# Weepingchestnut/SAVSR

Measured on NVIDIA B200. Metric: hr_mpix_per_s, higher is better.
Workload: dtype bf16

## Files before the change

savsr_b200/csrc/common.cuh:

```cuda
#pragma once

#include <cuda.h>
#include <cuda_bf16.h>
#include <cuda_fp16.h>
#include <cuda_runtime.h>
#include <stdint.h>
#include <stdio.h>
#include <string.h>

#include "../../include/savsr_b200.h"

namespace savsr {

void set_error(const char* fmt, ...);
int cuda_fail(cudaError_t e, const char* what);

#define SAVSR_CUDA(expr)                                   \
  do {                                                     \
    cudaError_t _e = (expr);                               \
    if (_e != cudaSuccess) return ::savsr::cuda_fail(_e, #expr); \
  } while (0)

#define SAVSR_REQUIRE(cond, ...)          \
  do {                                    \
    if (!(cond)) {                        \
      ::savsr::set_error(__VA_ARGS__);    \
      return 1;                           \
    }                                     \
  } while (0)

constexpr int kTileW = SAVSR_TILE_W;
constexpr int kTileH = SAVSR_TILE_H;
constexpr int kTileM = kTileW * kTileH;
constexpr int kC = 64;

}

struct savsr_ctx {
  int device;
  int sm_count;
  int cc_major, cc_minor;
  void* encode_tiled;
  int fmt;
  int opt[SAVSR_OPT_COUNT];
  uint32_t attr_mask;
  long long* conv_dbg;
};

namespace savsr {
enum AttrBit { kAttrIgemm = 0 , kAttrBigk = 8, kAttrKsta = 9, kAttrSatuHr = 10, kAttrOsaLinear = 11,
               kAttrFused = 12, kAttrBigk128 = 13, kAttrSatuHrBf16 = 14, kAttrWgrad = 15, kAttrWgradBatched = 16,
               kAttrOsaAssembleTrain = 17, kAttrOsaUnfoldBwd = 18, kAttrOsaChain = 19, kAttrOsaMatvec = 20 ,
               kAttrCaBackward = 23 };
template <class F>
inline int ensure_smem_attr(savsr_ctx* ctx, int bit, F func, size_t bytes) {
  if (ctx->attr_mask & (1u << bit)) return 0;
  SAVSR_CUDA(cudaFuncSetAttribute(func, cudaFuncAttributeMaxDynamicSharedMemorySize, static_cast<int>(bytes)));
  ctx->attr_mask |= 1u << bit;
  return 0;
}
template <class... KArgs, class... Args>
inline cudaError_t launch_k(bool pdl, void (*kernel)(KArgs...), dim3 grid, dim3 block, size_t smem, cudaStream_t st, Args&&... args) {
  cudaLaunchConfig_t cfg = {};
  cfg.gridDim = grid; cfg.blockDim = block; cfg.dynamicSmemBytes = smem; cfg.stream = st;
  cudaLaunchAttribute attr[1];
  attr[0].id = cudaLaunchAttributeProgrammaticStreamSerialization;
  attr[0].val.programmaticStreamSerializationAllowed = 1;
  cfg.attrs = attr; cfg.numAttrs = pdl ? 1 : 0;
  return cudaLaunchKernelEx(&cfg, kernel, static_cast<KArgs>(args)...);
}
struct DeviceGuard {
  int prev = -1;
  bool switched = false;
  explicit DeviceGuard(int device) {
    const bool known = cudaGetDevice(&prev) == cudaSuccess;
    const bool ok = cudaSetDevice(device) == cudaSuccess;
    switched = known && ok && prev != device;
  }
  ~DeviceGuard() { if (switched) cudaSetDevice(prev); }
};
}

struct savsr_arena {
  savsr_ctx* ctx;
  __nv_bfloat16* base;
  int nslots, batch, height, width;
  int tiles_x, tiles_y;
  CUtensorMap tm_tile;
  CUtensorMap tm_halo;
};

#ifdef __CUDACC__
namespace savsr {

__device__ __forceinline__ uint32_t smem_u32(const void* p) {
  return static_cast<uint32_t>(__cvta_generic_to_shared(p));
}

__device__ __forceinline__ uint32_t pack_h2(float lo, float hi, int fmt) {
  if (fmt) {
    __half2 v = __floats2half2_rn(lo, hi);
    return *reinterpret_cast<uint32_t*>(&v);
  }
  __nv_bfloat162 v = __floats2bfloat162_rn(lo, hi);
  return *reinterpret_cast<uint32_t*>(&v);
}
__device__ __forceinline__ float h_lo(uint32_t v, int fmt) {
  return fmt ? __half2float(__ushort_as_half(static_cast<unsigned short>(v & 0xffffu))) : __uint_as_float(v << 16);
}
__device__ __forceinline__ float h_hi(uint32_t v, int fmt) {
  return fmt ? __half2float(__ushort_as_half(static_cast<unsigned short>(v >> 16))) : __uint_as_float(v & 0xffff0000u);
}
__device__ __forceinline__ float h_to_float(uint16_t raw, int fmt) { return h_lo(raw, fmt); }
__device__ __forceinline__ uint16_t float_to_h(float x, int fmt) { return static_cast<uint16_t>(pack_h2(x, 0.f, fmt) & 0xffffu); }

__device__ __forceinline__ void bilinear_src(int dst, int in_size, int out_size, int& i0, int& i1, float& l1) {
  const float scale = static_cast<float>(in_size) / static_cast<float>(out_size);
  float src = scale * (static_cast<float>(dst) + 0.5f) - 0.5f;
  src = src < 0.f ? 0.f : src;
  i0 = static_cast<int>(src);
  i1 = i0 + (i0 < in_size - 1 ? 1 : 0);
  l1 = src - static_cast<float>(i0);
}

__device__ __forceinline__ bool elect_one() {
  uint32_t pred = 0;
  asm volatile(
      "{\n\t"
      ".reg .pred p;\n\t"
      "elect.sync _|p, 0xffffffff;\n\t"
      "selp.u32 %0, 1, 0, p;\n\t"
      "}\n"
      : "=r"(pred));
  return pred != 0;
}

__device__ __forceinline__ void named_barrier(int id, int count) {
  asm volatile("bar.sync %0, %1;" ::"r"(id), "r"(count) : "memory");
}
__device__ __forceinline__ void fence_proxy_async() { asm volatile("fence.proxy.async.shared::cta;" ::: "memory"); }
__device__ __forceinline__ void pdl_wait() { asm volatile("griddepcontrol.wait;" ::: "memory"); }
__device__ __forceinline__ void pdl_trigger() { asm volatile("griddepcontrol.launch_dependents;" ::: "memory"); }

__device__ __forceinline__ void mbar_init(uint64_t* bar, uint32_t count) {
  asm volatile("mbarrier.init.shared::cta.b64 [%0], %1;" ::"r"(smem_u32(bar)), "r"(count) : "memory");
}
__device__ __forceinline__ void fence_barrier_init() {
  asm volatile("fence.mbarrier_init.release.cluster;" ::: "memory");
}
__device__ __forceinline__ void mbar_expect_tx(uint64_t* bar, uint32_t bytes) {
  asm volatile("mbarrier.arrive.expect_tx.shared::cta.b64 _, [%0], %1;" ::"r"(smem_u32(bar)), "r"(bytes)
               : "memory");
}
__device__ __forceinline__ void mbar_arrive(uint64_t* bar) {
  asm volatile("mbarrier.arrive.shared::cta.b64 _, [%0];" ::"r"(smem_u32(bar)) : "memory");
}
__device__ __forceinline__ bool mbar_try_wait(uint64_t* bar, uint32_t parity) {
  uint32_t ok;
  asm volatile(
      "{\n\t"
      ".reg .pred p;\n\t"
      "mbarrier.try_wait.parity.shared::cta.b64 p, [%1], %2;\n\t"
      "selp.u32 %0, 1, 0, p;\n\t"
      "}\n"
      : "=r"(ok)
      : "r"(smem_u32(bar)), "r"(parity)
      : "memory");
  return ok != 0;
}
__device__ __forceinline__ void mbar_wait(uint64_t* bar, uint32_t parity) {
  uint32_t spins = 0;
  while (!mbar_try_wait(bar, parity)) {
    if (++spins > (1u << 26)) {
      printf("savsr: mbarrier timeout block %d thread %d bar %p parity %u\n", blockIdx.x, threadIdx.x,
             (void*)bar, parity);
      __trap();
    }
  }
}

__device__ __forceinline__ void prefetch_tensormap(const CUtensorMap* tm) {
  asm volatile("prefetch.tensormap [%0];" ::"l"(reinterpret_cast<uint64_t>(tm)) : "memory");
}
__device__ __forceinline__ void tma_load_4d(void* smem_dst, const CUtensorMap* tm, uint64_t* bar, int c, int x,
                                            int y, int img) {
  asm volatile(
      "cp.async.bulk.tensor.4d.shared::cluster.global.tile.mbarrier::complete_tx::bytes"
      " [%0], [%1, {%2, %3, %4, %5}], [%6];"
      ::"r"(smem_u32(smem_dst)), "l"(reinterpret_cast<uint64_t>(tm)), "r"(c), "r"(x), "r"(y), "r"(img),
      "r"(smem_u32(bar))
      : "memory");
}
__device__ __forceinline__ void tma_prefetch_4d(const CUtensorMap* tm, int c, int x, int y, int img) {
  asm volatile("cp.async.bulk.prefetch.tensor.4d.L2.global.tile [%0, {%1, %2, %3, %4}];"
               ::"l"(reinterpret_cast<uint64_t>(tm)), "r"(c), "r"(x), "r"(y), "r"(img)
               : "memory");
}
__device__ __forceinline__ void bulk_load(void* smem_dst, const void* gsrc, uint32_t bytes, uint64_t* bar) {
  asm volatile(
      "cp.async.bulk.shared::cluster.global.mbarrier::complete_tx::bytes [%0], [%1], %2, [%3];"
      ::"r"(smem_u32(smem_dst)), "l"(reinterpret_cast<uint64_t>(gsrc)), "r"(bytes), "r"(smem_u32(bar))
      : "memory");
}

__device__ __forceinline__ void tc_fence_before() { asm volatile("tcgen05.fence::before_thread_sync;" ::: "memory"); }
__device__ __forceinline__ void tc_fence_after() { asm volatile("tcgen05.fence::after_thread_sync;" ::: "memory"); }

template <int kCols>
__device__ __forceinline__ void tmem_alloc(uint32_t* smem_out) {
  asm volatile("tcgen05.alloc.cta_group::1.sync.aligned.shared::cta.b32 [%0], %1;" ::"r"(smem_u32(smem_out)),
               "n"(kCols)
               : "memory");
  asm volatile("tcgen05.relinquish_alloc_permit.cta_group::1.sync.aligned;" ::: "memory");
}
template <int kCols>
__device__ __forceinline__ void tmem_dealloc(uint32_t taddr) {
  asm volatile("tcgen05.dealloc.cta_group::1.sync.aligned.b32 %0, %1;" ::"r"(taddr), "n"(kCols) : "memory");
}

__device__ __forceinline__ uint64_t umma_desc_sw128(uint32_t saddr, uint32_t sbo_bytes, uint32_t base_offset) {
  uint64_t d = 0;
  d |= static_cast<uint64_t>((saddr >> 4) & 0x3fffu);
  d |= static_cast<uint64_t>((sbo_bytes >> 4) & 0x3fffu) << 32;
  d |= static_cast<uint64_t>(1) << 46;
  d |= static_cast<uint64_t>(base_offset & 7u) << 49;
  d |= static_cast<uint64_t>(2) << 61;
  return d;
}

__host__ __device__ constexpr uint32_t umma_idesc_f16(int n, int fmt) {
  return (1u << 4)
         | ((fmt ? 0u : 1u) << 7)
         | ((fmt ? 0u : 1u) << 10)
         | (static_cast<uint32_t>(n >> 3) << 17)
         | (static_cast<uint32_t>(128 >> 4) << 24);
}

__device__ __forceinline__ void umma_bf16(uint32_t tmem_d, uint64_t desc_a, uint64_t desc_b, uint32_t idesc,
                                          uint32_t accumulate) {
  asm volatile(
      "{\n\t"
      ".reg .pred p;\n\t"
      "setp.ne.b32 p, %4, 0;\n\t"
      "tcgen05.mma.cta_group::1.kind::f16 [%0], %1, %2, %3, p;\n\t"
      "}\n"
      ::"r"(tmem_d), "l"(desc_a), "l"(desc_b), "r"(idesc), "r"(accumulate)
      : "memory");
}
__device__ __forceinline__ void umma_commit(uint64_t* bar) {
  asm volatile("tcgen05.commit.cta_group::1.mbarrier::arrive::one.shared::cluster.b64 [%0];" ::"r"(smem_u32(bar))
               : "memory");
}

__host__ __device__ __forceinline__ int quad_row(int n) { return (n & 0x21) | (((n >> 1) & 3) << 3) | (((n >> 3) & 3) << 1); }

__device__ __forceinline__ void tmem_ld16(uint32_t taddr, uint32_t (&v)[16]) {
  asm volatile(
      "tcgen05.ld.sync.aligned.32x32b.x16.b32 "
      "{%0, %1, %2, %3, %4, %5, %6, %7, %8, %9, %10, %11, %12, %13, %14, %15}, [%16];"
      : "=r"(v[0]), "=r"(v[1]), "=r"(v[2]), "=r"(v[3]), "=r"(v[4]), "=r"(v[5]), "=r"(v[6]), "=r"(v[7]),
        "=r"(v[8]), "=r"(v[9]), "=r"(v[10]), "=r"(v[11]), "=r"(v[12]), "=r"(v[13]), "=r"(v[14]), "=r"(v[15])
      : "r"(taddr)
      : "memory");
}
__device__ __forceinline__ void tmem_ld_wait() { asm volatile("tcgen05.wait::ld.sync.aligned;" ::: "memory"); }

__device__ __forceinline__ void tmem_ld_16x256b_x4(uint32_t taddr, uint32_t (&v)[16]) {
  asm volatile(
      "tcgen05.ld.sync.aligned.16x256b.x4.b32 "
      "{%0, %1, %2, %3, %4, %5, %6, %7, %8, %9, %10, %11, %12, %13, %14, %15}, [%16];"
      : "=r"(v[0]), "=r"(v[1]), "=r"(v[2]), "=r"(v[3]), "=r"(v[4]), "=r"(v[5]), "=r"(v[6]), "=r"(v[7]),
        "=r"(v[8]), "=r"(v[9]), "=r"(v[10]), "=r"(v[11]), "=r"(v[12]), "=r"(v[13]), "=r"(v[14]), "=r"(v[15])
      : "r"(taddr)
      : "memory");
}

}
#endif
```

savsr_b200/csrc/small_ops.cu:

```cuda
#include "common.cuh"

namespace savsr {

__global__ void __launch_bounds__(256) pack_frames_kernel(const float* __restrict__ x, __nv_bfloat16* __restrict__ dst, int batch,
                                                          int t, int h, int w, int hp, int wp, int fmt) {
  const long npix = static_cast<long>(hp) * wp;
  const long total = static_cast<long>(batch) * npix * 8;
  for (long id = blockIdx.x * static_cast<long>(blockDim.x) + threadIdx.x; id < total; id += static_cast<long>(gridDim.x) * blockDim.x) {
    const int chunk = id & 7;
    const long pn = id >> 3;
    const long pix = pn % npix;
    const int n = pn / npix;
    const int py = pix / wp, px = pix % wp;
    const int ry = py < h ? py : 2 * h - 2 - py, rx = px < w ? px : 2 * w - 2 - px;
    float v[8];
#pragma unroll
    for (int e = 0; e < 8; ++e) {
      const int ch = chunk * 8 + e;
      v[e] = ch < 3 * t ? __ldg(x + ((static_cast<long>(n) * t * 3 + ch) * h + ry) * w + rx) : 0.f;
    }
    uint4 o;
    o.x = pack_h2(v[0], v[1], fmt); o.y = pack_h2(v[2], v[3], fmt); o.z = pack_h2(v[4], v[5], fmt); o.w = pack_h2(v[6], v[7], fmt);
    *reinterpret_cast<uint4*>(dst + (static_cast<long>(n) * npix + pix) * kC + chunk * 8) = o;
  }
}

constexpr int kMaxOsa = 4;
struct OsaLaunch {
  savsr_osa_params c[kMaxOsa];
  int nconvs, batch, npart, npix;
  float inv_h, inv_w;
  int fmt;
};
__host__ __device__ inline int osa_scratch_stride(int ci) { return 5 * ci + 192; }
__host__ __device__ inline int osa_off_h1(int ci) { return ci + 8; }
__host__ __device__ inline int osa_off_v2(int ci) { return 3 * ci + 8; }
__host__ __device__ inline int osa_off_att(int ci) { return 4 * ci + 8; }

__device__ __forceinline__ float sigmoidf_(float x) { return 1.f / (1.f + expf(-x)); }

constexpr int kOsaThreads = 1024;
__global__ void __launch_bounds__(kOsaThreads) osa_pool_kernel(const __grid_constant__ OsaLaunch L) {
  pdl_wait();
  pdl_trigger();
  const savsr_osa_params& c = L.c[blockIdx.z];
  const int s = blockIdx.x, n = blockIdx.y;
  if (s * 64 >= c.ci) return;
  __shared__ float red[16][64];
  const int ch = threadIdx.x & 63, part = threadIdx.x >> 6;
  const float* src = c.pool[s] + static_cast<long>(n) * L.npart * kC;
  float a0 = 0.f, a1 = 0.f;
  int q = part;
  for (; q + 16 < L.npart; q += 32) { a0 += src[q * kC + ch]; a1 += src[(q + 16) * kC + ch]; }
  if (q < L.npart) a0 += src[q * kC + ch];
  red[part][ch] = a0 + a1;
  __syncthreads();
  float* vin = c.scratch + static_cast<long>(n) * osa_scratch_stride(c.ci);
  if (part == 0) {
    float sum = 0.f;
#pragma unroll
    for (int k = 0; k < 16; ++k) sum += red[k][ch];
    vin[2 + s * 64 + ch] = sum / static_cast<float>(L.npix);
  }
  if (s == 0 && threadIdx.x == 0) { vin[0] = L.inv_h; vin[1] = L.inv_w; }
}

__global__ void __launch_bounds__(256) osa_linear_kernel(const __grid_constant__ OsaLaunch L, int layer) {
  pdl_wait();
  pdl_trigger();
  extern __shared__ float s_in[];
  const savsr_osa_params& c = L.c[blockIdx.y];
  const int rows = layer == 0 ? 2 * c.ci : c.ci;
  const int len = layer == 0 ? c.ci + 2 : 2 * c.ci;
  const int in_off = layer == 0 ? 0 : osa_off_h1(c.ci);
  const int out_off = layer == 0 ? osa_off_h1(c.ci) : osa_off_v2(c.ci);
  const float* W = layer == 0 ? c.r0_w : c.r2_w;
  const float* B = layer == 0 ? c.r0_b : c.r2_b;
  const int warp = threadIdx.x >> 5, lane = threadIdx.x & 31;
  if (blockIdx.x * 8 >= rows) return;
  const int stride = osa_scratch_stride(c.ci);
  const int per = (L.batch + gridDim.z - 1) / gridDim.z;
  const int n0 = blockIdx.z * per, n1 = min(L.batch, n0 + per);
  if (n0 >= n1) return;
  for (int i = threadIdx.x; i < (n1 - n0) * len; i += blockDim.x) {
    const int n = i / len, k = i - n * len;
    s_in[i] = c.scratch[static_cast<long>(n0 + n) * stride + in_off + k];
  }
  __syncthreads();
  const int row = blockIdx.x * 8 + warp;
  if (row >= rows) return;
  const float* wr = W + static_cast<long>(row) * len;
  float w[20];
#pragma unroll
  for (int j = 0; j < 20; ++j) w[j] = lane + 32 * j < len ? __ldg(wr + lane + 32 * j) : 0.f;
  const float bias = B[row];
  for (int n = n0; n < n1; ++n) {
    const float* in = s_in + (n - n0) * len;
    float acc = 0.f;
#pragma unroll
    for (int j = 0; j < 20; ++j) if (lane + 32 * j < len) acc += w[j] * in[lane + 32 * j];
#pragma unroll
    for (int off = 16; off >= 1; off >>= 1) acc += __shfl_xor_sync(0xffffffffu, acc, off);
    if (lane == 0) c.scratch[static_cast<long>(n) * stride + out_off + row] = fmaxf(acc + bias, 0.f);
  }
}

constexpr int kAsmMaxSamples = 8;
__global__ void __launch_bounds__(256) osa_assemble_kernel(const __grid_constant__ OsaLaunch L) {
  const savsr_osa_params& c = L.c[blockIdx.y];
  __shared__ float z_s[kAsmMaxSamples][32];
  __shared__ float att_s[kAsmMaxSamples][64 * SAVSR_MAX_SRC + 64 + 9 + 8];
  const int per = (L.batch + gridDim.z - 1) / gridDim.z;
  const int n0 = blockIdx.z * per, n1 = min(L.batch, n0 + per);
  if (n0 >= n1 || blockIdx.x * blockDim.x >= c.co * c.ci) return;
  const int ns = n1 - n0;
  const int warp = threadIdx.x >> 5, lane = threadIdx.x & 31;
  const int stride = osa_scratch_stride(c.ci);
  const int nout = c.ci + c.co + 9 + 8;
  for (int a = warp; a < c.att; a += 8) {
    float wr[10];
#pragma unroll
    for (int j = 0; j < 10; ++j) wr[j] = lane + 32 * j < c.ci ? __ldg(c.fc_w + a * c.ci + lane + 32 * j) : 0.f;
    const float bs = c.bn_scale[a], bh = c.bn_shift[a];
    for (int n = 0; n < ns; ++n) {
      const float* v2 = c.scratch + static_cast<long>(n0 + n) * stride + osa_off_v2(c.ci);
      float acc = 0.f;
#pragma unroll
      for (int j = 0; j < 10; ++j) if (lane + 32 * j < c.ci) acc += wr[j] * v2[lane + 32 * j];
#pragma unroll
      for (int off = 16; off >= 1; off >>= 1) acc += __shfl_xor_sync(0xffffffffu, acc, off);
      if (lane == 0) z_s[n][a] = fmaxf(acc * bs + bh, 0.f);
    }
  }
  __syncthreads();
  for (int j = threadIdx.x; j < nout; j += blockDim.x) {
    const float* w;
    float b;
    if (j < c.ci) { w = c.ch_w + j * c.att; b = c.ch_b[j]; }
    else if (j < c.ci + c.co) { w = c.fl_w + (j - c.ci) * c.att; b = c.fl_b[j - c.ci]; }
    else if (j < c.ci + c.co + 9) { w = c.sp_w + (j - c.ci - c.co) * c.att; b = c.sp_b[j - c.ci - c.co]; }
    else { w = c.kn_w + (j - c.ci - c.co - 9) * c.att; b = c.kn_b[j - c.ci - c.co - 9]; }
    float wv[32];
#pragma unroll
    for (int a = 0; a < 32; ++a) wv[a] = a < c.att ? __ldg(w + a) : 0.f;
    const bool sig = j < c.ci + c.co + 9;
    for (int n = 0; n < ns; ++n) {
      float acc = b;
#pragma unroll
      for (int a = 0; a < 32; ++a) if (a < c.att) acc += wv[a] * z_s[n][a];
      att_s[n][j] = sig ? sigmoidf_(acc) : acc;
    }
  }
  __syncthreads();
  if (threadIdx.x < ns) {
    float* ka = att_s[threadIdx.x] + c.ci + c.co + 9;
    float mx = ka[0];
    for (int k = 1; k < 8; ++k) mx = fmaxf(mx, ka[k]);
    float e[8], sum = 0.f;
    for (int k = 0; k < 8; ++k) { e[k] = expf(ka[k] - mx); sum += e[k]; }
    for (int k = 0; k < 8; ++k) ka[k] = e[k] / sum;
  }
  __syncthreads();
  if (blockIdx.x == 0) {
    for (int r = threadIdx.x; r < ns * nout; r += blockDim.x) {
      const int n = r / nout, j = r - n * nout;
      c.scratch[static_cast<long>(n0 + n) * stride + osa_off_att(c.ci) + j] = att_s[n][j];
    }
  }
  const int idx = blockIdx.x * blockDim.x + threadIdx.x;
  if (idx >= c.co * c.ci) return;
  const int i = idx % c.ci, o = idx / c.ci;
  float bk[8][9];
  const long per_k = static_cast<long>(c.co) * c.ci * 9;
#pragma unroll
  for (int k = 0; k < 8; ++k) {
    const float* src = c.bank + k * per_k + (static_cast<long>(o) * c.ci + i) * 9;
#pragma unroll
    for (int t = 0; t < 9; ++t) bk[k][t] = __ldg(src + t);
  }
  const int s = i >> 6, kk = i & 63;
  const long sample_elems = static_cast<long>(c.co) * c.ci * 9;
  const int row = quad_row(o);
  const int inner = row * 64 + ((((kk >> 3) ^ (row & 7)) << 3) | (kk & 7));
  for (int n = 0; n < ns; ++n) {
    const float* att = att_s[n];
    const float ca = att[i], fa = att[c.ci + o];
    const float* sa = att + c.ci + c.co;
    const float* ka = sa + 9;
    uint16_t* dst = static_cast<uint16_t*>(c.packed) + (n0 + n) * sample_elems;
#pragma unroll
    for (int t = 0; t < 9; ++t) {
      float acc = 0.f;
#pragma unroll
      for (int k = 0; k < 8; ++k) acc += ka[k] * bk[k][t];
      dst[static_cast<long>(s * 9 + t) * 4096 + inner] = float_to_h(acc * sa[t] * ca * fa, L.fmt);
    }
  }
}

struct CaParams {
  const __nv_bfloat16* t;
  const __nv_bfloat16* x;
  __nv_bfloat16* dst;
  const float* pool;
  const float *w1, *b1, *w2, *b2;
  float* y;
  int npart;
  int fmt;
  long npix;
};
__global__ void __launch_bounds__(1024) ca_vector_kernel(const CaParams p) {
  pdl_wait();
  pdl_trigger();
  __shared__ float red[16][64];
  __shared__ float mean[64];
  __shared__ float hid[4];
  const int n = blockIdx.x;
  const int ch = threadIdx.x & 63, part = threadIdx.x >> 6;
  const float* src = p.pool + static_cast<long>(n) * p.npart * kC;
  float a0 = 0.f, a1 = 0.f;
  int q = part;
  for (; q + 16 < p.npart; q += 32) { a0 += src[q * kC + ch]; a1 += src[(q + 16) * kC + ch]; }
  if (q < p.npart) a0 += src[q * kC + ch];
  red[part][ch] = a0 + a1;
  __syncthreads();
  if (part == 0) {
    float sum = 0.f;
#pragma unroll
    for (int k = 0; k < 16; ++k) sum += red[k][ch];
    mean[ch] = sum / static_cast<float>(p.npix);
  }
  __syncthreads();
  if (threadIdx.x < 4) {
    float a = p.b1[threadIdx.x];
    for (int i = 0; i < 64; ++i) a += p.w1[threadIdx.x * 64 + i] * mean[i];
    hid[threadIdx.x] = fmaxf(a, 0.f);
  }
  __syncthreads();
  if (threadIdx.x < 64) {
    float a = p.b2[threadIdx.x];
#pragma unroll
    for (int i = 0; i < 4; ++i) a += p.w2[threadIdx.x * 4 + i] * hid[i];
    p.y[n * 64 + threadIdx.x] = sigmoidf_(a);
  }
}
__global__ void __launch_bounds__(256) ca_scale_residual_kernel(const CaParams p) {
  pdl_wait();
  pdl_trigger();
  __shared__ float ys[64];
  const int n = blockIdx.y;
  if (threadIdx.x < 64) ys[threadIdx.x] = p.y[n * 64 + threadIdx.x];
  __syncthreads();
  const long chunks = p.npix * 8;
  const uint4* tt = reinterpret_cast<const uint4*>(p.t + static_cast<long>(n) * p.npix * kC);
  const uint4* xx = reinterpret_cast<const uint4*>(p.x + static_cast<long>(n) * p.npix * kC);
  uint4* dd = reinterpret_cast<uint4*>(p.dst + static_cast<long>(n) * p.npix * kC);
  for (long id = blockIdx.x * static_cast<long>(blockDim.x) + threadIdx.x; id < chunks;
       id += static_cast<long>(gridDim.x) * blockDim.x) {
    const int c0 = (id & 7) * 8;
    const uint4 a = tt[id], b = xx[id];
    uint4 o;
    o.x = pack_h2(h_lo(b.x, p.fmt) + h_lo(a.x, p.fmt) * ys[c0 + 0], h_hi(b.x, p.fmt) + h_hi(a.x, p.fmt) * ys[c0 + 1], p.fmt);
    o.y = pack_h2(h_lo(b.y, p.fmt) + h_lo(a.y, p.fmt) * ys[c0 + 2], h_hi(b.y, p.fmt) + h_hi(a.y, p.fmt) * ys[c0 + 3], p.fmt);
    o.z = pack_h2(h_lo(b.z, p.fmt) + h_lo(a.z, p.fmt) * ys[c0 + 4], h_hi(b.z, p.fmt) + h_hi(a.z, p.fmt) * ys[c0 + 5], p.fmt);
    o.w = pack_h2(h_lo(b.w, p.fmt) + h_lo(a.w, p.fmt) * ys[c0 + 6], h_hi(b.w, p.fmt) + h_hi(a.w, p.fmt) * ys[c0 + 7], p.fmt);
    dd[id] = o;
  }
}

template <bool kPool, bool kProj>
__global__ void __launch_bounds__(256) mask_conv16_kernel(const float* __restrict__ in, const float* __restrict__ w,
                                                          const float* __restrict__ b, const float* __restrict__ wf,
                                                          float* __restrict__ out, int h2, int w2) {
  __shared__ __align__(16) float w_s[9 * 16 * 16 + 36 * 4];
  __shared__ float wf_s[9 * 16];
  for (int i = threadIdx.x; i < 9 * 256; i += blockDim.x) {
    const int co = i & 15, ci = (i >> 4) & 15, tap = i >> 8;
    w_s[i + (i >> 6) * 4] = w[(co * 16 + ci) * 9 + tap];
  }
  if (kProj) {
    for (int i = threadIdx.x; i < 144; i += blockDim.x) wf_s[i] = wf[(i & 15) * 9 + (i >> 4)];
  }
  __syncthreads();
  const int n = blockIdx.y;
  const int q = threadIdx.x & 3;
  const long npix2 = static_cast<long>(h2) * w2;
  const long pix = blockIdx.x * static_cast<long>(blockDim.x >> 2) + (threadIdx.x >> 2);
  const bool live = pix < npix2;
  const int py = live ? pix / w2 : 0, px = live ? pix % w2 : 0;
  float acc[16];
#pragma unroll
  for (int o = 0; o < 16; ++o) acc[o] = 0.f;
  const int wfull = 2 * w2;
  const float* base = kPool ? in + static_cast<long>(n) * (4 * npix2) * 16 : in + static_cast<long>(n) * npix2 * 16;
#pragma unroll
  for (int tap = 0; tap < 9; ++tap) {
    const int sy = py + tap / 3 - 1, sx = px + tap % 3 - 1;
    if (!live || sy < 0 || sy >= h2 || sx < 0 || sx >= w2) continue;
    float4 a;
    if (kPool) {
      const float4 q0 = *reinterpret_cast<const float4*>(base + (static_cast<long>(2 * sy) * wfull + 2 * sx) * 16 + 4 * q);
      const float4 q1 = *reinterpret_cast<const float4*>(base + (static_cast<long>(2 * sy) * wfull + 2 * sx + 1) * 16 + 4 * q);
      const float4 q2 = *reinterpret_cast<const float4*>(base + (static_cast<long>(2 * sy + 1) * wfull + 2 * sx) * 16 + 4 * q);
      const float4 q3 = *reinterpret_cast<const float4*>(base + (static_cast<long>(2 * sy + 1) * wfull + 2 * sx + 1) * 16 + 4 * q);
      a.x = 0.25f * ((q0.x + q1.x) + (q2.x + q3.x)); a.y = 0.25f * ((q0.y + q1.y) + (q2.y + q3.y));
      a.z = 0.25f * ((q0.z + q1.z) + (q2.z + q3.z)); a.w = 0.25f * ((q0.w + q1.w) + (q2.w + q3.w));
    } else {
      a = *reinterpret_cast<const float4*>(base + (static_cast<long>(sy) * w2 + sx) * 16 + 4 * q);
    }
    const float av[4] = {a.x, a.y, a.z, a.w};
#pragma unroll
    for (int c = 0; c < 4; ++c) {
      const float4* wr = reinterpret_cast<const float4*>(w_s + (tap * 16 + 4 * q + c) * 16 + (tap * 4 + q) * 4);
#pragma unroll
      for (int o4 = 0; o4 < 4; ++o4) {
        const float4 wv = wr[o4];
        acc[4 * o4 + 0] += av[c] * wv.x; acc[4 * o4 + 1] += av[c] * wv.y;
        acc[4 * o4 + 2] += av[c] * wv.z; acc[4 * o4 + 3] += av[c] * wv.w;
      }
    }
  }
#pragma unroll
  for (int off = 2, cnt = 8; off >= 1; off >>= 1, cnt >>= 1) {
    const bool upper = (q & off) != 0;
#pragma unroll
    for (int i = 0; i < cnt; ++i) {
      const float send = upper ? acc[i] : acc[i + cnt];
      const float keep = upper ? acc[i + cnt] : acc[i];
      acc[i] = keep + __shfl_xor_sync(0xffffffffu, send, off);
    }
  }
  float o4v[4];
#pragma unroll
  for (int i = 0; i < 4; ++i) o4v[i] = fmaxf(acc[i] + b[4 * q + i], 0.f);
  if (!kProj) {
    if (live) *reinterpret_cast<float4*>(out + (static_cast<long>(n) * npix2 + pix) * 16 + 4 * q) = make_float4(o4v[0], o4v[1], o4v[2], o4v[3]);
  } else {
    float d[9];
#pragma unroll
    for (int t = 0; t < 9; ++t) {
      float v = 0.f;
#pragma unroll
      for (int i = 0; i < 4; ++i) v += wf_s[t * 16 + 4 * q + i] * o4v[i];
      v += __shfl_xor_sync(0xffffffffu, v, 1);
      v += __shfl_xor_sync(0xffffffffu, v, 2);
      d[t] = v;
    }
    if (live && q < 3) {
      float* dst = out + (static_cast<long>(n) * npix2 + pix) * 12 + 4 * q;
      *reinterpret_cast<float4*>(dst) = q == 0 ? make_float4(d[0], d[1], d[2], d[3])
                                     : q == 1 ? make_float4(d[4], d[5], d[6], d[7]) : make_float4(d[8], 0.f, 0.f, 0.f);
    }
  }
}

__global__ void __launch_bounds__(256) mask_final_kernel(const float* __restrict__ d, const float* __restrict__ b,
                                                         float* __restrict__ mask, int h2, int w2) {
  const int n = blockIdx.y;
  const int H = 2 * h2, W = 2 * w2;
  const long npix = static_cast<long>(H) * W;
  const long pix = blockIdx.x * static_cast<long>(blockDim.x) + threadIdx.x;
  if (pix >= npix) return;
  const int py = pix / W, px = pix % W;
  const float* base = d + static_cast<long>(n) * h2 * w2 * 12;
  float acc = b[0];
#pragma unroll
  for (int tap = 0; tap < 9; ++tap) {
    const int sy = py + tap / 3 - 1, sx = px + tap % 3 - 1;
    if (sy < 0 || sy >= H || sx < 0 || sx >= W) continue;
    float fy = 0.5f * (static_cast<float>(sy) + 0.5f) - 0.5f;
    float fx = 0.5f * (static_cast<float>(sx) + 0.5f) - 0.5f;
    fy = fy < 0.f ? 0.f : fy;
    fx = fx < 0.f ? 0.f : fx;
    const int y0 = static_cast<int>(fy), x0 = static_cast<int>(fx);
    const int y1 = y0 + (y0 < h2 - 1 ? 1 : 0), x1 = x0 + (x0 < w2 - 1 ? 1 : 0);
    const float ly = fy - y0, lx = fx - x0;
    const float v00 = base[(static_cast<long>(y0) * w2 + x0) * 12 + tap], v01 = base[(static_cast<long>(y0) * w2 + x1) * 12 + tap];
    const float v10 = base[(static_cast<long>(y1) * w2 + x0) * 12 + tap], v11 = base[(static_cast<long>(y1) * w2 + x1) * 12 + tap];
    acc += (1.f - ly) * ((1.f - lx) * v00 + lx * v01) + ly * ((1.f - lx) * v10 + lx * v11);
  }
  mask[static_cast<long>(n) * npix + pix] = sigmoidf_(acc);
}

__device__ __forceinline__ float y_of_u8(int b, int g, int r) {
  const double d = (static_cast<double>(static_cast<float>(b) / 255.f) * 24.966 + static_cast<double>(static_cast<float>(g) / 255.f) * 128.553) +
                   static_cast<double>(static_cast<float>(r) / 255.f) * 65.481 + 16.0;
  return static_cast<float>(d / 255.) * 255.f;
}
__global__ void __launch_bounds__(256) img_metrics_kernel(const float* __restrict__ sr, const float* __restrict__ gt, int H, int W,
                                                          uint8_t* __restrict__ bgr, double* __restrict__ sse) {
  const int n = blockIdx.y;
  const long npix = static_cast<long>(H) * W;
  const float* s = sr + static_cast<long>(n) * 3 * npix;
  const float* g = gt ? gt + static_cast<long>(n) * 3 * npix : nullptr;
  double acc = 0.0;
  for (long pix = blockIdx.x * static_cast<long>(blockDim.x) + threadIdx.x; pix < npix; pix += static_cast<long>(gridDim.x) * blockDim.x) {
    int q[3], qg[3];
#pragma unroll
    for (int c = 0; c < 3; ++c) {
      q[c] = __float2int_rn(fminf(fmaxf(s[c * npix + pix], 0.f), 1.f) * 255.0f);
      if (g) qg[c] = __float2int_rn(fminf(fmaxf(g[c * npix + pix], 0.f), 1.f) * 255.0f);
    }
    if (bgr) {
      uint8_t* o = bgr + (static_cast<long>(n) * npix + pix) * 3;
      o[0] = static_cast<uint8_t>(q[2]); o[1] = static_cast<uint8_t>(q[1]); o[2] = static_cast<uint8_t>(q[0]);
    }
    if (g) {
      const double d = static_cast<double>(y_of_u8(q[2], q[1], q[0])) - static_cast<double>(y_of_u8(qg[2], qg[1], qg[0]));
      acc += d * d;
    }
  }
  if (sse) {
    __shared__ double red[8];
#pragma unroll
    for (int off = 16; off >= 1; off >>= 1) acc += __shfl_xor_sync(0xffffffffu, acc, off);
    if ((threadIdx.x & 31) == 0) red[threadIdx.x >> 5] = acc;
    __syncthreads();
    if (threadIdx.x == 0) {
      double t = 0.0;
      for (int i = 0; i < 8; ++i) t += red[i];
      sse[static_cast<long>(n) * gridDim.x + blockIdx.x] = t;
    }
  }
}

}

using namespace savsr;

struct SsimParams {
  const float* sr;
  const float* gt;
  double* partials;
  int H, W, bx, by;
  double k[11];
};
__global__ void __launch_bounds__(256) ssim_y_kernel(const __grid_constant__ SsimParams p) {
  __shared__ double y1[26][27], y2[26][27];
  __shared__ double red[8];
  const int n = blockIdx.z;
  const long npix = static_cast<long>(p.H) * p.W;
  const float* s = p.sr + static_cast<long>(n) * 3 * npix;
  const float* g = p.gt + static_cast<long>(n) * 3 * npix;
  const int oy0 = blockIdx.y * 16, ox0 = blockIdx.x * 16;
  for (int i = threadIdx.x; i < 26 * 26; i += 256) {
    const int r = i / 26, c = i - r * 26;
    const int y = oy0 + r, x = ox0 + c;
    double a = 0.0, b = 0.0;
    if (y < p.H && x < p.W) {
      const long pix = static_cast<long>(y) * p.W + x;
      int q[3], qg[3];
#pragma unroll
      for (int ch = 0; ch < 3; ++ch) {
        q[ch] = __float2int_rn(fminf(fmaxf(s[ch * npix + pix], 0.f), 1.f) * 255.0f);
        qg[ch] = __float2int_rn(fminf(fmaxf(g[ch * npix + pix], 0.f), 1.f) * 255.0f);
      }
      a = static_cast<double>(y_of_u8(q[2], q[1], q[0]));
      b = static_cast<double>(y_of_u8(qg[2], qg[1], qg[0]));
    }
    y1[r][c] = a; y2[r][c] = b;
  }
  __syncthreads();
  const int ty = threadIdx.x >> 4, tx = threadIdx.x & 15;
  double val = 0.0;
  if (oy0 + ty < p.H - 10 && ox0 + tx < p.W - 10) {
    double mu1 = 0.0, mu2 = 0.0, s11 = 0.0, s22 = 0.0, s12 = 0.0;
    for (int i = 0; i < 11; ++i) {
#pragma unroll
      for (int j = 0; j < 11; ++j) {
        const double w = p.k[i] * p.k[j];
        const double a = y1[ty + i][tx + j], b = y2[ty + i][tx + j];
        mu1 += w * a; mu2 += w * b;
        s11 += w * (a * a); s22 += w * (b * b); s12 += w * (a * b);
      }
    }
    const double c1 = (0.01 * 255) * (0.01 * 255), c2 = (0.03 * 255) * (0.03 * 255);
    const double mu1_sq = mu1 * mu1, mu2_sq = mu2 * mu2, mu12 = mu1 * mu2;
    val = ((2 * mu12 + c1) * (2 * (s12 - mu12) + c2)) / ((mu1_sq + mu2_sq + c1) * ((s11 - mu1_sq) + (s22 - mu2_sq) + c2));
  }
#pragma unroll
  for (int off = 16; off >= 1; off >>= 1) val += __shfl_xor_sync(0xffffffffu, val, off);
  if ((threadIdx.x & 31) == 0) red[threadIdx.x >> 5] = val;
  __syncthreads();
  if (threadIdx.x == 0) {
    double t = 0.0;
    for (int i = 0; i < 8; ++i) t += red[i];
    p.partials[(static_cast<long>(n) * p.by + blockIdx.y) * p.bx + blockIdx.x] = t;
  }
}

extern "C" int savsr_pack_frames(savsr_ctx* ctx, savsr_arena* arena, const float* x, int t, int h, int w, int dst_slot, savsr_stream st) {
  SAVSR_REQUIRE(ctx && arena && x, "savsr_pack_frames: null pointer");
  DeviceGuard guard(ctx->device);
  SAVSR_REQUIRE(t >= 1 && 3 * t <= kC, "savsr_pack_frames: %d frames do not fit 64 channels", t);
  SAVSR_REQUIRE(h >= 2 && w >= 2, "savsr_pack_frames: LR frame %dx%d too small for reflect padding", h, w);
  SAVSR_REQUIRE(arena->height == h + (h & 1) && arena->width == w + (w & 1),
                "savsr_pack_frames: arena %dx%d is not the even-padded size of %dx%d", arena->height, arena->width, h, w);
  SAVSR_REQUIRE(dst_slot >= 0 && dst_slot < arena->nslots, "savsr_pack_frames: slot %d out of range", dst_slot);
  if (arena->batch == 0) return 0;
  const long npix = static_cast<long>(arena->height) * arena->width;
  const long total = arena->batch * npix * 8;
  const int blocks = static_cast<int>((total + 255) / 256 < 4096 ? (total + 255) / 256 : 4096);
  pack_frames_kernel<<<blocks, 256, 0, static_cast<cudaStream_t>(st)>>>(x, arena->base + static_cast<long>(dst_slot) * arena->batch * npix * kC,
                                                                       arena->batch, t, h, w, arena->height, arena->width, ctx->fmt);
  SAVSR_CUDA(cudaGetLastError());
  return 0;
}

namespace savsr {
int osa_prologue_front(savsr_ctx* ctx, const savsr_osa_params* convs, int nconvs, int batch, int npart, int npix, float inv_scale_h,
                       float inv_scale_w, cudaStream_t st) {
  OsaLaunch L;
  memset(&L, 0, sizeof(L));
  int max_ci = 0;
  for (int i = 0; i < nconvs; ++i) {
    L.c[i] = convs[i];
    max_ci = convs[i].ci > max_ci ? convs[i].ci : max_ci;
  }
  L.nconvs = nconvs; L.batch = batch; L.npart = npart; L.npix = npix;
  L.inv_h = inv_scale_h; L.inv_w = inv_scale_w;
  L.fmt = ctx->fmt;
  (void)launch_k(ctx->opt[SAVSR_OPT_PDL] != 0, osa_pool_kernel, dim3(max_ci / 64, batch, nconvs), dim3(kOsaThreads), 0, st, L);
  const int lin_split = batch >= 12 ? 3 : (batch >= 4 ? 2 : 1);
  const size_t lin_smem = static_cast<size_t>((batch + lin_split - 1) / lin_split) * 2 * max_ci * sizeof(float);
  SAVSR_REQUIRE(lin_smem <= 200 * 1024, "savsr_osa_prologue: batch %d too large for the routing kernel's shared memory", batch);
  if (lin_smem > 48 * 1024) {
    if (int rc = ensure_smem_attr(ctx, kAttrOsaLinear, osa_linear_kernel, 200 * 1024)) return rc;
  }
  (void)launch_k(ctx->opt[SAVSR_OPT_PDL] != 0, osa_linear_kernel, dim3((2 * max_ci + 7) / 8, nconvs, lin_split), dim3(256), lin_smem, st, L, 0);
  (void)launch_k(ctx->opt[SAVSR_OPT_PDL] != 0, osa_linear_kernel, dim3((max_ci + 7) / 8, nconvs, lin_split), dim3(256), lin_smem, st, L, 1);
  SAVSR_CUDA(cudaGetLastError());
  return 0;
}
}

extern "C" int savsr_osa_prologue(savsr_ctx* ctx, const savsr_osa_params* convs, int nconvs, int batch, int npart,
                                  int npix, float inv_scale_h, float inv_scale_w, savsr_stream st_) {
  SAVSR_REQUIRE(ctx && convs, "savsr_osa_prologue: null pointer");
  DeviceGuard guard(ctx->device);
  SAVSR_REQUIRE(nconvs >= 0 && nconvs <= kMaxOsa, "savsr_osa_prologue: nconvs %d out of range [0,%d]", nconvs, kMaxOsa);
  if (nconvs == 0 || batch == 0) return 0;
  cudaStream_t st = static_cast<cudaStream_t>(st_);
  OsaLaunch L;
  memset(&L, 0, sizeof(L));
  int max_ci = 0;
  for (int i = 0; i < nconvs; ++i) {
    const savsr_osa_params& c = convs[i];
    SAVSR_REQUIRE(c.ci > 0 && c.ci % 64 == 0 && c.ci <= 64 * SAVSR_MAX_SRC, "savsr_osa_prologue: conv %d ci %d unsupported", i, c.ci);
    SAVSR_REQUIRE(c.co == 64, "savsr_osa_prologue: conv %d co %d unsupported (64 only)", i, c.co);
    SAVSR_REQUIRE(c.att > 0 && c.att <= 32, "savsr_osa_prologue: conv %d attention channels %d out of range", i, c.att);
    SAVSR_REQUIRE(c.bank && c.r0_w && c.r0_b && c.r2_w && c.r2_b && c.fc_w && c.bn_scale && c.bn_shift && c.ch_w && c.ch_b &&
                  c.fl_w && c.fl_b && c.sp_w && c.sp_b && c.kn_w && c.kn_b && c.scratch && c.packed,
                  "savsr_osa_prologue: conv %d has a null parameter pointer", i);
    for (int s = 0; s < c.ci / 64; ++s) SAVSR_REQUIRE(c.pool[s], "savsr_osa_prologue: conv %d source %d has no pool buffer", i, s);
    L.c[i] = c;
    max_ci = c.ci > max_ci ? c.ci : max_ci;
  }
  L.nconvs = nconvs; L.batch = batch; L.npart = npart; L.npix = npix;
  L.inv_h = inv_scale_h; L.inv_w = inv_scale_w;
  L.fmt = ctx->fmt;
  if (int rc = osa_prologue_front(ctx, convs, nconvs, batch, npart, npix, inv_scale_h, inv_scale_w, st)) return rc;
  int asm_split = batch >= 16 ? 4 : (batch >= 6 ? 2 : 1);
  while ((batch + asm_split - 1) / asm_split > kAsmMaxSamples) ++asm_split;
  osa_assemble_kernel<<<dim3((64 * max_ci + 255) / 256, nconvs, asm_split), 256, 0, st>>>(L);
  SAVSR_CUDA(cudaGetLastError());
  return 0;
}

extern "C" int savsr_ca_scale_residual(savsr_ctx* ctx, savsr_arena* arena, int t_slot, int x_slot, int dst_slot,
                                       const float* pool, int npart, const float* w1, const float* b1, const float* w2,
                                       const float* b2, float* y_scratch, savsr_stream st) {
  SAVSR_REQUIRE(ctx && arena && pool && w1 && b1 && w2 && b2 && y_scratch, "savsr_ca_scale_residual: null pointer");
  DeviceGuard guard(ctx->device);
  SAVSR_REQUIRE(t_slot >= 0 && t_slot < arena->nslots && x_slot >= 0 && x_slot < arena->nslots && dst_slot >= 0 &&
                dst_slot < arena->nslots, "savsr_ca_scale_residual: slot out of range");
  CaParams p;
  p.npix = static_cast<long>(arena->height) * arena->width;
  const long img = p.npix * kC * arena->batch;
  p.t = arena->base + t_slot * img;
  p.x = arena->base + x_slot * img;
  p.dst = arena->base + dst_slot * img;
  p.fmt = ctx->fmt; p.pool = pool; p.npart = npart; p.w1 = w1; p.b1 = b1; p.w2 = w2; p.b2 = b2; p.y = y_scratch;
  long blocks = (p.npix * 8 + 255) / 256;
  const long cap = 8L * ctx->sm_count / (arena->batch > 0 ? arena->batch : 1) + 1;
  if (blocks > cap) blocks = cap;
  if (arena->batch == 0) return 0;
  (void)launch_k(ctx->opt[SAVSR_OPT_PDL] != 0, ca_vector_kernel, dim3(arena->batch), dim3(1024), 0, static_cast<cudaStream_t>(st), p);
  (void)launch_k(ctx->opt[SAVSR_OPT_PDL] != 0, ca_scale_residual_kernel, dim3(static_cast<unsigned>(blocks), arena->batch), dim3(256), 0, static_cast<cudaStream_t>(st), p);
  SAVSR_CUDA(cudaGetLastError());
  return 0;
}

extern "C" int savsr_osadapt_mask(savsr_ctx* ctx, const float* in16, int batch, int height, int width, const float* wa,
                                  const float* ba, const float* wb, const float* bb, const float* wc, const float* bc,
                                  float* half0, float* half1, float* mask, savsr_stream st_) {
  SAVSR_REQUIRE(ctx && in16 && wa && ba && wb && bb && wc && bc && half0 && half1 && mask, "savsr_osadapt_mask: null pointer");
  DeviceGuard guard(ctx->device);
  SAVSR_REQUIRE(height % 2 == 0 && width % 2 == 0, "savsr_osadapt_mask: size %dx%d must be even (pad_spatial)", height, width);
  if (batch == 0) return 0;
  cudaStream_t st = static_cast<cudaStream_t>(st_);
  const int h2 = height / 2, w2 = width / 2;
  const long npix2 = static_cast<long>(h2) * w2;
  dim3 g2(static_cast<unsigned>((npix2 + 63) / 64), batch);
  mask_conv16_kernel<true, false><<<g2, 256, 0, st>>>(in16, wa, ba, nullptr, half0, h2, w2);
  mask_conv16_kernel<false, true><<<g2, 256, 0, st>>>(half0, wb, bb, wc, half1, h2, w2);
  dim3 g1(static_cast<unsigned>((4 * npix2 + 255) / 256), batch);
  mask_final_kernel<<<g1, 256, 0, st>>>(half1, bc, mask, h2, w2);
  SAVSR_CUDA(cudaGetLastError());
  return 0;
}

static long img_metrics_grid(const savsr_ctx* ctx, int height, int width) {
  const long npix = static_cast<long>(height) * width;
  long blocks = (npix + 255) / 256;
  if (blocks > 4L * ctx->sm_count) blocks = 4L * ctx->sm_count;
  return blocks;
}

extern "C" int savsr_img_metrics_blocks(const savsr_ctx* ctx, int height, int width) {
  return (ctx && height > 0 && width > 0) ? static_cast<int>(img_metrics_grid(ctx, height, width)) : 0;
}

extern "C" int savsr_img_metrics(savsr_ctx* ctx, const float* sr, const float* gt, int batch, int height, int width, uint8_t* bgr_u8,
                                 double* sse_y, savsr_stream st_) {
  SAVSR_REQUIRE(ctx && sr, "savsr_img_metrics: null pointer");
  DeviceGuard guard(ctx->device);
  SAVSR_REQUIRE(batch >= 0 && height > 0 && width > 0, "savsr_img_metrics: bad shape");
  SAVSR_REQUIRE(!sse_y || gt, "savsr_img_metrics: sse_y requested without a ground-truth frame");
  if (batch == 0) return 0;
  cudaStream_t st = static_cast<cudaStream_t>(st_);
  const long blocks = img_metrics_grid(ctx, height, width);
  img_metrics_kernel<<<dim3(static_cast<unsigned>(blocks), batch), 256, 0, st>>>(sr, gt, height, width, bgr_u8, sse_y);
  SAVSR_CUDA(cudaGetLastError());
  return 0;
}

extern "C" int savsr_ssim_y_blocks(int height, int width) {
  if (height < 11 || width < 11) return 0;
  return ((height - 10 + 15) / 16) * ((width - 10 + 15) / 16);
}

extern "C" int savsr_ssim_y(savsr_ctx* ctx, const float* sr, const float* gt, int batch, int height, int width, double* partials,
                            savsr_stream st) {
  SAVSR_REQUIRE(ctx && sr && gt && partials, "savsr_ssim_y: null pointer");
  DeviceGuard guard(ctx->device);
  SAVSR_REQUIRE(batch >= 0 && height >= 11 && width >= 11, "savsr_ssim_y: frames of %dx%d are smaller than the 11x11 window", height, width);
  if (batch == 0) return 0;
  SsimParams p;
  p.sr = sr; p.gt = gt; p.partials = partials; p.H = height; p.W = width;
  p.bx = (width - 10 + 15) / 16; p.by = (height - 10 + 15) / 16;
  double sum = 0.0;
  for (int i = 0; i < 11; ++i) { p.k[i] = exp(-((i - 5.0) * (i - 5.0)) / (2.0 * 1.5 * 1.5)); sum += p.k[i]; }
  for (int i = 0; i < 11; ++i) p.k[i] /= sum;
  ssim_y_kernel<<<dim3(p.bx, p.by, batch), 256, 0, static_cast<cudaStream_t>(st)>>>(p);
  SAVSR_CUDA(cudaGetLastError());
  return 0;
}
```

savsr_b200/engine.py:

```python
from __future__ import annotations

import os

import ctypes as C
from typing import Callable, Dict, List, Optional, Sequence, Tuple

import numpy as np
import torch

from . import _capi as K

BN_EPS = 1e-5


def normalize_scale(scale) -> Tuple[float, float]:
    if isinstance(scale, (int, float)):
        return (scale, scale)
    s = tuple(scale)
    if len(s) != 2:
        raise ValueError(f"scale must be a number or a (s_h, s_w) pair, got {scale!r}")
    return (s[0], s[1])


def get_hw(h: int, w: int, scale) -> Tuple[int, int]:
    s = normalize_scale(scale)
    return round(h * s[0]), round(w * s[1])


_contexts: Dict[int, K.Context] = {}


def context(device_index: int) -> K.Context:
    if device_index not in _contexts:
        c = K.Context(device_index)
        if os.environ.get("SAVSR_BIGK_ALL") is not None:
            c.set_option(K.OPT_BIGK_ALL, int(os.environ["SAVSR_BIGK_ALL"] != "0"))
        if os.environ.get("SAVSR_BIGK_ISSUERS") is not None:
            c.set_option(K.OPT_BIGK_ISSUERS, int(os.environ["SAVSR_BIGK_ISSUERS"]))
        if os.environ.get("SAVSR_PDL") is not None:
            c.set_option(K.OPT_PDL, int(os.environ["SAVSR_PDL"] != "0"))
        _contexts[device_index] = c
    return _contexts[device_index]


class pdl:

    def __init__(self, ctx: K.Context, on: bool):
        self.ctx = ctx
        env = os.environ.get("SAVSR_PDL")
        self.on = int(on if env is None else env != "0")

    def __enter__(self):
        self.prev = self.ctx.lib.savsr_ctx_get_option(self.ctx.handle, K.OPT_PDL)
        self.ctx.set_option(K.OPT_PDL, self.on)
        return self

    def __exit__(self, *exc):
        self.ctx.set_option(K.OPT_PDL, max(self.prev, 0))
        return False


class WeightStore:

    def __init__(self, version: tuple = ()):
        self.version = version
        self.cache: Dict[tuple, torch.Tensor] = {}

    def get(self, key: tuple, make: Callable[[], torch.Tensor]) -> torch.Tensor:
        t = self.cache.get(key)
        if t is None:
            t = self.cache[key] = make()
        return t


class _Slots:

    def __init__(self):
        self.free: List[int] = []
        self.n = 0

    def get(self) -> int:
        if self.free:
            return self.free.pop()
        self.n += 1
        return self.n - 1

    def get_many(self, k: int) -> List[int]:
        return [self.get() for _ in range(k)]

    def get_contiguous(self, k: int) -> int:
        s = self.n
        self.n += k
        return s

    def put(self, *slots: int) -> None:
        self.free.extend(slots)


def satu_hr_compose(P: Dict[str, torch.Tensor], device: torch.device):
    g = lambda name: P[name].detach().to(device, torch.float64)
    u = "upsample"
    Wf = g(u + ".fusion.weight").view(64, 128)
    bf = g(u + ".fusion.bias")
    Wt = g("tail.weight").permute(2, 3, 0, 1).reshape(27, 64)
    comb = Wt @ Wf
    Wcs, Wcf = comb[:, :64], comb[:, 64:]
    We = g(u + ".weight_expand").view(4, 64, 8).permute(1, 0, 2).reshape(64, 32)
    Wv = Wcf @ We
    Wc = g(u + ".weight_compress").reshape(32, 64)
    zb = torch.zeros(32, dtype=torch.float64, device=device)
    zb[:27] = Wt @ bf
    return Wc.float(), Wcf.float().contiguous(), Wcs.float().contiguous(), Wv.float(), zb.float()


def satu_hr_pack(parts, fmt: int, device: torch.device) -> torch.Tensor:
    dt = torch.float16 if fmt == K.FMT_FP16 else torch.bfloat16
    n = torch.arange(32, device=device).view(32, 1)
    pos = torch.arange(8, device=device).view(1, 8) ^ (n & 7)
    tiles = []
    for m in parts[:4]:
        full = torch.zeros(32, 64, device=device)
        full[:m.shape[0], :m.shape[1]] = m
        src = full.to(dt).view(32, 8, 8)
        tile = torch.zeros_like(src)
        tile.scatter_(1, pos.view(32, 8, 1).expand(32, 8, 8), src)
        tiles.append(tile.reshape(-1))
    return torch.cat(tiles).view(torch.uint8).contiguous()


class Plan:
    def __init__(self, params: Dict[str, torch.Tensor], batch: int, h: int, w: int, scale, device: torch.device,
                 conv_impl: str = "tap", num_frame: int = 7, taps: Optional[Sequence[str]] = None, precision: str = "bf16",
                 store: Optional[WeightStore] = None):
        if device.type != "cuda":
            raise K.SavsrError("savsr_b200 runs on CUDA (sm_100a) only; there is no CPU fallback")
        if num_frame != 7:
            raise NotImplementedError("only the shipped 7-frame configuration is implemented")
        if h < 2 or w < 2:
            raise ValueError(f"LR frames must be at least 2x2, got {h}x{w}")
        self.device = device
        self.ctx = context(device.index if device.index is not None else torch.cuda.current_device())
        self.lib = self.ctx.lib
        self.impl = K.IMPL_NAMES[conv_impl]
        if precision not in K.FMT_NAMES:
            raise ValueError(f"precision must be one of {sorted(K.FMT_NAMES)}, got {precision!r}")
        self.fmt = K.FMT_NAMES[precision]
        self.B, self.h, self.w, self.t = batch, h, w, num_frame
        self.scale = normalize_scale(scale)
        self.hp, self.wp = h + (h & 1), w + (w & 1)
        self.H, self.W = get_hw(h, w, self.scale)
        self.P = params
        self._keep: List[object] = []
        self._pack_src: List[torch.Tensor] = []
        self.ops: List[Callable[[int], int]] = []
        self.op_meta: List[Tuple[str, float, int, str]] = []
        self.n_launches = 0
        self.taps = set(taps or ())
        self.tap_bufs: Dict[str, torch.Tensor] = {}
        self.graph: Optional[torch.cuda.CUDAGraph] = None
        self.store = store if store is not None else WeightStore()
        self.nbytes = 0
        self._pool_cache: Dict[str, int] = {}
        self._osa_cache: Dict[str, Tuple[K.OsaParams, int, int]] = {}
        self.cplan: Optional[K.CPlan] = K.CPlan(self.ctx) if hasattr(K, "CPlan") and hasattr(self.lib, "savsr_plan_create") else None
        self._recorded = 0
        with torch.cuda.device(device), torch.no_grad():
            self.ctx.set_format(self.fmt)
            self._build()
            if self.cplan is not None:
                if self._recorded == len(self.ops):
                    K.check(self.lib.savsr_plan_set_io(self.cplan.handle, self.x_in.data_ptr(), self.x_in.numel() * 4, self.out.data_ptr(),
                                                       self.out.numel() * 4, self.fmt))
                else:
                    self.cplan = None

    def _buf(self, *shape, dtype=torch.float32) -> torch.Tensor:
        t = torch.empty(*shape, dtype=dtype, device=self.device)
        self._keep.append(t)
        self.nbytes += t.numel() * t.element_size()
        return t

    def _p(self, name: str) -> torch.Tensor:
        t = self.P[name]
        if t.device != self.device or t.dtype != torch.float32 or not t.is_contiguous():
            t = t.detach().to(self.device, torch.float32).contiguous()
        self._keep.append(t)
        return t

    def _ptr(self, name: str) -> int:
        return self._p(name).data_ptr()

    def _derived(self, key, make: Callable[[], torch.Tensor]) -> torch.Tensor:
        return self.store.get(("derived", key), lambda: make().detach().to(self.device, torch.float32).contiguous())

    def _dev(self, key, make: Callable[[], torch.Tensor]) -> int:
        return self._derived(key, make).data_ptr()

    def _packp(self, name: str) -> int:
        return self._pack(name, lambda: self._p(name))

    def _pack(self, key, make: Callable[[], torch.Tensor], n_tile: int = 64, co_pad: Optional[int] = None,
              rows: int = K.ROWS_QUAD) -> int:
        def build() -> torch.Tensor:
            w = make().detach().to(self.device, torch.float32).contiguous()
            co_real, ci, ks, _ = w.shape
            co = co_pad or co_real
            out = torch.empty(self.lib.savsr_packed_weight_bytes(co, ci, ks), dtype=torch.uint8, device=self.device)
            K.check(self.lib.savsr_pack_conv_weight(w.data_ptr(), co_real, co, ci, ks, n_tile, self.fmt, rows, out.data_ptr(),
                                                    torch.cuda.current_stream(self.device).cuda_stream))
            self._pack_src.append(w)
            return out
        return self.store.get(("packed", key, n_tile, co_pad, rows, self.fmt), build).data_ptr()

    def _emit(self, fn: Callable[[int], int], launches: int = 1, kind: str = "other", flops: float = 0.0,
              detail: str = "", rec: Optional[Callable[[object], int]] = None) -> None:
        self.ops.append(fn)
        self.op_meta.append((kind, flops, launches, detail))
        self.n_launches += launches
        if rec is not None and self.cplan is not None:
            K.check(rec(self.cplan.handle))
            self._recorded += 1

    def _group(self, src: Sequence[int], dst: int, weight: int, bias: int = 0, act: int = K.ACT_NONE, slope: float = 0.2,
               res1: int = -1, res2: int = -1, res2_scale: float = 0.0, wstride: int = 0, mask: int = 0, pool: int = 0,
               aux: int = 0, src_channels: int = 0) -> K.ConvGroup:
        g = K.ConvGroup()
        for i, s in enumerate(src):
            g.src_slot[i] = s
        g.nsrc = len(src)
        g.dst_slot, g.res1_slot, g.res2_slot, g.res2_scale = dst, res1, res2, res2_scale
        g.act, g.slope = act, slope
        g.weight, g.weight_sample_stride = weight, wstride
        g.bias, g.mask, g.pool, g.aux_dst = bias or None, mask or None, pool or None, aux or None
        g.src_channels = src_channels
        return g

    def _conv(self, arena: K.Arena, groups: Sequence[K.ConvGroup], ksize: int = 3, n_tile: int = 64,
              dst_mode: int = K.DST_ARENA, alg_ci: Optional[Sequence[int]] = None, alg_co: Optional[int] = None,
              kind: Optional[str] = None) -> None:
        arr = (K.ConvGroup * len(groups))(*groups)
        self._keep.append(arr)
        lib, ctx, ah, n, impl = self.lib, self.ctx.handle, arena.handle, len(groups), self.impl
        co = alg_co if alg_co is not None else (64 if n_tile == 64 else 16)
        ci = list(alg_ci) if alg_ci is not None else [64 * g.nsrc for g in groups]
        flops = 2.0 * self.B * arena.height * arena.width * co * ksize * ksize * sum(ci)
        osa = any(g.weight_sample_stride != 0 for g in groups)
        self._emit(lambda st: lib.savsr_conv(ctx, ah, arr, n, ksize, n_tile, dst_mode, impl, st),
                   kind=kind or f"conv{ksize}x{ksize}_n{n_tile}", flops=flops,
                   detail=f"g{n}s{groups[0].nsrc}" + ("osa" if osa else ""),
                   rec=lambda cp: lib.savsr_plan_add_conv(cp, ah, arr, n, ksize, n_tile, dst_mode, impl))

    def _tap(self, name: str, arena: str, slot: int) -> None:
        if name not in self.taps:
            return
        a = self.lr
        buf = self._buf(self.B, 64, a.height, a.width)
        self.tap_bufs[name] = buf
        lib, ah, ptr = self.lib, a.handle, buf.data_ptr()
        self._emit(lambda st: lib.savsr_arena_export(ah, slot, ptr, st), kind="debug_tap", rec=lambda cp: lib.savsr_plan_add_arena_export(cp, ah, slot, ptr))

    def _osa_params(self, prefix: str, nsrc: int, pools: Sequence[int]) -> Tuple[K.OsaParams, int, int]:
        if prefix in self._osa_cache:
            return self._osa_cache[prefix]
        ci, co = 64 * nsrc, 64
        att = max(int(ci * 0.0625), 16)
        a = prefix + ".attention"
        def bn_s():
            return self._p(a + ".bn.weight") / torch.sqrt(self._p(a + ".bn.running_var") + BN_EPS)

        def bn_b():
            return self._p(a + ".bn.bias") - self._p(a + ".bn.running_mean") * bn_s()
        o = K.OsaParams()
        o.ci, o.co, o.att = ci, co, att
        o.bank = self._ptr(prefix + ".weight")
        o.r0_w, o.r0_b = self._ptr(prefix + ".scale_routing.0.weight"), self._ptr(prefix + ".scale_routing.0.bias")
        o.r2_w, o.r2_b = self._ptr(prefix + ".scale_routing.2.weight"), self._ptr(prefix + ".scale_routing.2.bias")
        o.fc_w = self._ptr(a + ".fc.weight")
        o.bn_scale, o.bn_shift = self._dev(a + ".bn_scale", bn_s), self._dev(a + ".bn_shift", bn_b)
        o.ch_w, o.ch_b = self._ptr(a + ".channel_fc.weight"), self._ptr(a + ".channel_fc.bias")
        o.fl_w, o.fl_b = self._ptr(a + ".filter_fc.weight"), self._ptr(a + ".filter_fc.bias")
        o.sp_w, o.sp_b = self._ptr(a + ".spatial_fc.weight"), self._ptr(a + ".spatial_fc.bias")
        o.kn_w, o.kn_b = self._ptr(a + ".kernel_fc.weight"), self._ptr(a + ".kernel_fc.bias")
        for i, pp in enumerate(pools):
            o.pool[i] = pp
        scratch = self._buf(self.B, 5 * ci + 192)
        packed = self._buf(self.B, co * ci * 9 * 2, dtype=torch.uint8)
        o.scratch, o.packed = scratch.data_ptr(), packed.data_ptr()
        self.osa_scratch[prefix] = scratch
        self._osa_cache[prefix] = (o, packed.data_ptr(), co * ci * 9 * 2)
        return self._osa_cache[prefix]

    def _osa_prologue(self, convs: Sequence[K.OsaParams]) -> None:
        arr = (K.OsaParams * len(convs))(*convs)
        self._keep.append(arr)
        inv_h = float(np.float32(1.0) / np.float32(self.scale[0]))
        inv_w = float(np.float32(1.0) / np.float32(self.scale[1]))
        lib, ctx, n, B = self.lib, self.ctx.handle, len(convs), self.B
        npart, npix = self.lr.tiles * 4, self.hp * self.wp
        self._emit(lambda st: lib.savsr_osa_prologue(ctx, arr, n, B, npart, npix, inv_h, inv_w, st), launches=4, kind="osa_prologue",
                   rec=lambda cp: lib.savsr_plan_add_osa_prologue(cp, arr, n, B, npart, npix, inv_h, inv_w))

    def _pool(self, key: str) -> int:
        if key not in self._pool_cache:
            self._pool_cache[key] = self._buf(self.B, self.lr.tiles * 4, 64).data_ptr()
        return self._pool_cache[key]

    def _residual_block(self, prefixes: Sequence[str], xs: Sequence[Sequence[int]], outs: Sequence[Sequence[int]],
                        tmp: Sequence[Sequence[int]], base: Sequence[int]) -> None:
        lr = self.lr
        nfr = len(xs[0])
        use_os = (prefixes[0] + ".osconv.weight") in self.P
        L = K.ACT_LRELU
        pools = [[self._pool(f"{p}.conv0.{i}") if use_os else 0 for i in range(nfr)] for p in prefixes]
        self._conv(lr, [self._group([xs[d][i]], tmp[d][i], self._packp(f"{p}.conv0.{i}.weight"),
                                    self._ptr(f"{p}.conv0.{i}.bias"), act=L, pool=pools[d][i])
                        for d, p in enumerate(prefixes) for i in range(nfr)])
        if use_os:
            osa = [self._osa_params(p + ".osconv", nfr, pools[d]) for d, p in enumerate(prefixes)]
            self._osa_prologue([o[0] for o in osa])
            self._conv(lr, [self._group(tmp[d], base[d], osa[d][1], act=L, wstride=osa[d][2]) for d in range(len(prefixes))])
        else:
            self._conv(lr, [self._group(tmp[d], base[d], self._packp(p + ".conv1.weight"), self._ptr(p + ".conv1.bias"), act=L)
                            for d, p in enumerate(prefixes)], ksize=1)
        self._conv(lr, [self._group([base[d], tmp[d][i]], outs[d][i], self._packp(f"{p}.conv2.{i}.weight"),
                                    self._ptr(f"{p}.conv2.{i}.bias"), act=L, res1=xs[d][i])
                        for d, p in enumerate(prefixes) for i in range(nfr)])

    def _build(self) -> None:
        P, B, t = self.P, self.B, self.t
        lib, ctx = self.lib, self.ctx.handle
        L = K.ACT_LRELU
        self.osa_scratch: Dict[str, torch.Tensor] = {}
        nf = 64
        sl = _Slots()
        zero = sl.get()
        FR = sl.get()
        dirs = ("f2p_win", "p2f_win")
        n_it = t - 3 + 1
        F = [[sl.get() for _ in range(n_it)] for _ in dirs]
        S0 = [sl.get_many(2) for _ in dirs]
        S1 = [sl.get_many(3) for _ in dirs]
        S2 = [sl.get_many(3) for _ in dirs]
        T = [sl.get_many(3) for _ in dirs]
        Bs = [sl.get() for _ in dirs]
        pool_free = [s for d in range(2) for s in (S0[d] + S1[d] + S2[d] + T[d])] + Bs
        extra_needed = 5 + 5 + 5 + 1 + 2 + 1 + 6 + 2
        while len(pool_free) < extra_needed:
            pool_free.append(sl.get())
        self.n_lr_slots = sl.n
        self.arena_lr_t = self._buf(self.n_lr_slots * B, self.hp, self.wp, 64, dtype=torch.bfloat16)
        self.arena_lr_t.zero_()
        self.lr = K.Arena(self.ctx, self.arena_lr_t.data_ptr(), self.n_lr_slots, B, self.hp, self.wp)
        lr = self.lr
        self.x_in = self._buf(B, t, 3, self.h, self.w)
        self.out = self._buf(B, 3, self.H, self.W)
        xin = self.x_in.data_ptr()

        lrh0, hh0, ww0 = lr.handle, self.h, self.w
        self._emit(lambda st: lib.savsr_pack_frames(ctx, lrh0, xin, t, hh0, ww0, FR, st), kind="pack_frames",
                   rec=lambda cp: lib.savsr_plan_add_pack_frames(cp, lrh0, xin, t, hh0, ww0, FR))
        hpast = [zero, zero]
        for idx in range(n_it):
            centre = [t - 1 - 1 - idx, idx + 1]
            fgroups = []
            for d, p in enumerate(dirs):
                c = centre[d]

                def wc(p=p, c=c):
                    wz = torch.zeros(64, 64, 3, 3, device=self.device)
                    wz[:, 3 * c:3 * c + 3] = self._p(p + ".conv_c.weight")
                    return wz

                def ws(p=p, c=c):
                    wz = torch.zeros(64, 64, 3, 3, device=self.device)
                    wsup = self._p(p + ".conv_sup.weight")
                    wz[:, 3 * (c - 1):3 * (c - 1) + 3] = wsup[:, 0:3]
                    wz[:, 3 * (c + 1):3 * (c + 1) + 3] = wsup[:, 3:6]
                    return wz
                fgroups.append(self._group([FR], S0[d][0], self._pack((p, "conv_c@", c), wc), self._ptr(p + ".conv_c.bias"), act=L, src_channels=32))
                fgroups.append(self._group([FR], S0[d][1], self._pack((p, "conv_sup@", c), ws), self._ptr(p + ".conv_sup.bias"), act=L, src_channels=32))
            self._conv(lr, fgroups, alg_ci=[3, 6, 3, 6])
            cur = [[S0[d][0], S0[d][1], hpast[d]] for d in range(2)]
            sets = [S1, S2]
            for j in range(4):
                nxt = sets[j % 2]
                self._residual_block([f"{p}.blocks.{j}" for p in dirs], cur, nxt, T, Bs)
                cur = [list(nxt[d]) for d in range(2)]
            self._conv(lr, [self._group(cur[d], F[d][idx], self._packp(p + ".merge.weight"), self._ptr(p + ".merge.bias"))
                            for d, p in enumerate(dirs)])
            hpast = [F[0][idx], F[1][idx]]
        self._tap("f2p_last", "lr", F[0][n_it - 1])
        self._tap("p2f_last", "lr", F[1][n_it - 1])

        free = list(pool_free)
        take = lambda k: [free.pop() for _ in range(k)]
        Gx, Gy, T5 = take(5), take(5), take(5)
        B5, = take(1)
        M = take(2)
        A, = take(1)
        p2 = "h_win.0"
        self._conv(lr, [self._group([F[0][n_it - 1 - i], F[1][i]], Gx[i], self._packp(f"{p2}.conv_h.{i}.weight"),
                                    self._ptr(f"{p2}.conv_h.{i}.bias"), act=L) for i in range(5)])
        cur5, nxt5 = Gx, Gy
        for j in range(2):
            self._residual_block([f"{p2}.blocks.{j}"], [cur5], [nxt5], [T5], [B5])
            cur5, nxt5 = nxt5, cur5
        wm = self._packp(p2 + ".merge.weight")
        half = 5 * 9 * 8192
        bm = self._p(p2 + ".merge.bias")
        self._conv(lr, [self._group(cur5, M[k], wm + k * half, bm[64 * k:].data_ptr()) for k in range(2)])
        self._tap("h_win0", "lr", M[0]); self._tap("h_win1", "lr", M[1])
        self._conv(lr, [self._group(M, A, self._packp("h_win_conv_h.weight"), self._ptr("h_win_conv_h.bias"), act=L)])
        self._tap("align", "lr", A)
        free += Gx + Gy + T5 + [B5] + M

        gamma = float(self._p("gamma").item())
        X0, X1, T1, T2, R, Hs = take(6)
        in16 = self._buf(B, self.hp * self.wp, 16)
        half0 = self._buf(B, (self.hp // 2) * (self.wp // 2), 16)
        half1 = self._buf(B, (self.hp // 2) * (self.wp // 2), 16)
        maskb = self._buf(B, self.hp * self.wp)
        ca_y = self._buf(B, 64).data_ptr()
        npart = lr.tiles * 4
        lrh = lr.handle
        h_cur = A
        for gi in range(4):
            x, xa, xb = h_cur, X0, X1
            for r in range(8):
                pr = f"RG.{gi}.residual_group.{r}.rcab"
                self._conv(lr, [self._group([x], T1, self._packp(pr + ".0.weight"), self._ptr(pr + ".0.bias"), act=K.ACT_RELU)])
                pl = self._pool(pr + ".2")
                self._conv(lr, [self._group([T1], T2, self._packp(pr + ".2.weight"), self._ptr(pr + ".2.bias"), pool=pl)])
                w1, b1 = self._ptr(pr + ".3.attention.1.weight"), self._ptr(pr + ".3.attention.1.bias")
                w2, b2 = self._ptr(pr + ".3.attention.3.weight"), self._ptr(pr + ".3.attention.3.bias")
                self._emit(lambda st, x=x, xa=xa, pl=pl, w1=w1, b1=b1, w2=w2, b2=b2:
                           lib.savsr_ca_scale_residual(ctx, lrh, T2, x, xa, pl, npart, w1, b1, w2, b2, ca_y, st),
                           launches=2, kind="ca_scale_residual",
                           rec=lambda cp, x=x, xa=xa, pl=pl, w1=w1, b1=b1, w2=w2, b2=b2:
                           lib.savsr_plan_add_ca_scale_residual(cp, lrh, T2, x, xa, pl, npart, w1, b1, w2, b2, ca_y))
                x, xa, xb = xa, xb, xa
            plr = self._pool(f"RG.{gi}.conv")
            self._conv(lr, [self._group([x], R, self._packp(f"RG.{gi}.conv.weight"), self._ptr(f"RG.{gi}.conv.bias"),
                                        res1=h_cur, pool=plr)])
            self._tap(f"rg{gi}", "lr", R)
            pa = f"adapt.{gi}"
            m = pa + ".mask"

            def fold(conv: str, bn: str):
                def sc():
                    return self._p(bn + ".weight") / torch.sqrt(self._p(bn + ".running_var") + BN_EPS)
                return (lambda: self._p(conv + ".weight") * sc().view(-1, 1, 1, 1),
                        lambda: (self._p(conv + ".bias") - self._p(bn + ".running_mean")) * sc() + self._p(bn + ".bias"))
            w0, b0 = fold(m + ".0", m + ".1")
            wa, ba = fold(m + ".4", m + ".5")
            wb, bb = fold(m + ".7", m + ".8")
            wc, bc = fold(m + ".11", m + ".12")
            self._conv(lr, [self._group([R], 0, self._pack(m + ".0+bn", w0, n_tile=16), self._dev(m + ".0+bn.bias", b0), act=K.ACT_RELU,
                                        aux=in16.data_ptr())], n_tile=16, dst_mode=K.DST_AUX16)
            args = (ctx, in16.data_ptr(), B, self.hp, self.wp, self._dev(m + ".4+bn.w", wa), self._dev(m + ".4+bn.b", ba),
                    self._dev(m + ".7+bn.w", wb), self._dev(m + ".7+bn.b", bb), self._dev(m + ".11+bn.w", wc), self._dev(m + ".11+bn.b", bc),
                    half0.data_ptr(), half1.data_ptr(), maskb.data_ptr())
            self._emit(lambda st, args=args: lib.savsr_osadapt_mask(*args, st), launches=3, kind="osadapt_mask",
                       rec=lambda cp, args=args: lib.savsr_plan_add_osadapt_mask(cp, *args[1:]))
            osa = self._osa_params(pa + ".adapt", 1, [plr])
            self._osa_prologue([osa[0]])
            self._conv(lr, [self._group([R], Hs, osa[1], wstride=osa[2], mask=maskb.data_ptr(), res1=R, res2=A, res2_scale=gamma)])
            self._tap(f"adapt{gi}", "lr", Hs)
            h_cur = Hs
        TR, = take(1)
        self._conv(lr, [self._group([h_cur], TR, self._packp("conv_last.weight"), self._ptr("conv_last.bias"), res1=A)])
        self._tap("trunk", "lr", TR)

        u = "upsample"
        wkp = self._pack(u + ".kernel_conv.tapmajor",
                         lambda: self._p(u + ".kernel_conv.0.weight").view(64, 25, 64).permute(1, 0, 2).reshape(1600, 64, 1, 1))
        bkp = self._dev(u + ".kernel_conv.tapmajor.bias", lambda: self._p(u + ".kernel_conv.0.bias").view(64, 25).t().contiguous())
        STA, = take(1)
        lrh, hh, ww = lr.handle, self.h, self.w
        kflops = 2.0 * B * self.hp * self.wp * 64 * 1600
        self._emit(lambda st: lib.savsr_satu_kconv_sta(ctx, lrh, A, TR, STA, hh, ww, wkp, bkp, 0.1, st), kind="satu_kconv_sta",
                   flops=kflops, rec=lambda cp: lib.savsr_plan_add_satu_kconv_sta(cp, lrh, A, TR, STA, hh, ww, wkp, bkp, 0.1))
        self._tap("satu_sta", "lr", STA)
        sw = K.SatuWeights()
        sw.body0_w, sw.body0_b = self._ptr(u + ".body.0.weight"), self._ptr(u + ".body.0.bias")
        sw.body2_w, sw.body2_b = self._ptr(u + ".body.2.weight"), self._ptr(u + ".body.2.bias")
        sw.routing_w, sw.routing_b = self._ptr(u + ".routing.0.weight"), self._ptr(u + ".routing.0.bias")
        sw.offset_w, sw.offset_b = self._ptr(u + ".offset.weight"), self._ptr(u + ".offset.bias")
        sw.st_offset_w, sw.st_offset_b = self._ptr(u + ".st_offset.weight"), self._ptr(u + ".st_offset.bias")
        sw.compress, sw.expand = self._ptr(u + ".weight_compress"), self._ptr(u + ".weight_expand")
        self._keep.append(sw)
        H, W = self.H, self.W
        self.rel_y, self.rel_x = self._buf(H), self._buf(W)
        self.base_y, self.base_x = self._buf(H), self._buf(W)
        self.cell_y, self.cell_x = self._buf(H, dtype=torch.int32), self._buf(W, dtype=torch.int32)
        self.corner_y, self.corner_x = self._buf(H, dtype=torch.int32), self._buf(W, dtype=torch.int32)
        self.table = self._buf(H * W, 8)
        K.check(lib.savsr_satu_index(ctx, C.byref(sw), self.h, self.w, H, W, float(self.scale[0]), float(self.scale[1]),
                                     self.rel_y.data_ptr(), self.rel_x.data_ptr(), self.cell_y.data_ptr(), self.cell_x.data_ptr(),
                                     self.base_y.data_ptr(), self.base_x.data_ptr(), self.corner_y.data_ptr(),
                                     self.corner_x.data_ptr(), self.table.data_ptr(), self._stream().cuda_stream))
        tab, by, bx = self.table.data_ptr(), self.base_y.data_ptr(), self.base_x.data_ptr()
        hw = self.store.get(("satu_hr_weights", self.fmt), lambda: satu_hr_pack(satu_hr_compose(P, self.device), self.fmt, self.device))
        zb = self._dev("satu_hr.zbias", lambda: satu_hr_compose(P, self.device)[4])
        tb = self._ptr("tail.bias")
        hwp, outp, cen = hw.data_ptr(), self.out.data_ptr(), t // 2
        hr_flops = 2.0 * B * self.H * self.W * (64 * 32 + 32 * 64 + 128 * 64 + 64 * 3 * 9)
        self._emit(lambda st: lib.savsr_satu_hr(ctx, lrh, TR, STA, hh, ww, H, W, tab, by, bx, hwp, zb, tb, xin, t, cen, outp, st),
                   kind="satu_hr", flops=hr_flops,
                   rec=lambda cp: lib.savsr_plan_add_satu_hr(cp, lrh, TR, STA, hh, ww, H, W, tab, by, bx, hwp, zb, tb, xin, t, cen, outp))
        self.satu_extra_bytes_per_sample = 2 * 64 * self.hp * self.wp * 2
        self._stream().synchronize()
        self._pack_src.clear()

    def _stream(self) -> "torch.cuda.Stream":
        return torch.cuda.current_stream(self.device)

    def run(self) -> None:
        with torch.cuda.device(self.device), pdl(self.ctx, self.B <= 2):
            self.ctx.set_format(self.fmt)
            st = self._stream().cuda_stream
            if self.cplan is not None:
                K.check(self.lib.savsr_plan_run(self.cplan.handle, st))
                return
            for op in self.ops:
                rc = op(st)
                if rc:
                    K.check(rc)

    def run_profiled(self, detail: bool = False) -> Dict[str, Dict[str, float]]:
        with torch.cuda.device(self.device):
            self.ctx.set_format(self.fmt)
            stream = self._stream()
            st = stream.cuda_stream
            evs = []
            for op in self.ops:
                e0, e1 = torch.cuda.Event(enable_timing=True), torch.cuda.Event(enable_timing=True)
                e0.record(stream)
                rc = op(st)
                e1.record(stream)
                if rc:
                    K.check(rc)
                evs.append((e0, e1))
            stream.synchronize()
        out: Dict[str, Dict[str, float]] = {}
        for (kind, flops, launches, tag), (e0, e1) in zip(self.op_meta, evs):
            d = out.setdefault(f"{kind}:{tag}" if (detail and tag) else kind, dict(ms=0.0, flops=0.0, ops=0, launches=0))
            d["ms"] += e0.elapsed_time(e1); d["flops"] += flops; d["ops"] += 1; d["launches"] += launches
        return out

    def time_ops_graph(self, select: Callable[[str, str], bool], reps: int = 5) -> Dict[str, float]:
        idx = [i for i, (kind, _, _, detail) in enumerate(self.op_meta) if select(kind, detail)]
        if not idx:
            return dict(ms=0.0, flops=0.0, launches=0, ops=0)
        with torch.cuda.device(self.device):
            self.ctx.set_format(self.fmt)
            torch.cuda.synchronize(self.device)
            g = torch.cuda.CUDAGraph()
            with torch.cuda.graph(g, stream=torch.cuda.Stream(self.device)):
                st = torch.cuda.current_stream(self.device).cuda_stream
                for i in idx:
                    rc = self.ops[i](st)
                    if rc:
                        K.check(rc)
            stream = self._stream()
            g.replay()
            e0, e1 = torch.cuda.Event(enable_timing=True), torch.cuda.Event(enable_timing=True)
            e0.record(stream)
            for _ in range(reps):
                g.replay()
            e1.record(stream)
            stream.synchronize()
        return dict(ms=e0.elapsed_time(e1) / reps, flops=sum(self.op_meta[i][1] for i in idx), launches=sum(self.op_meta[i][2] for i in idx), ops=len(idx))

    def capture(self) -> None:
        if self.graph is not None:
            return
        with torch.cuda.device(self.device):
            self.run()
            torch.cuda.synchronize(self.device)
            g = torch.cuda.CUDAGraph()
            with torch.cuda.graph(g, stream=torch.cuda.Stream(self.device)):
                self.run()
            self.graph = g

    def run_graph(self) -> None:
        if self.graph is None:
            self.capture()
        with torch.cuda.device(self.device):
            self.graph.replay()

    def forward_into(self, x: torch.Tensor, out: torch.Tensor, graph: bool = True) -> None:
        with torch.cuda.device(self.device):
            self.x_in.copy_(x, non_blocking=True)
            if graph:
                self.run_graph()
            else:
                self.run()
            out.copy_(self.out, non_blocking=True)

    def activation_absmax(self) -> float:
        dt = torch.float16 if self.fmt == K.FMT_FP16 else torch.bfloat16
        with torch.cuda.device(self.device):
            peak = float(torch.linalg.vector_norm(self.arena_lr_t.view(dt).reshape(-1), ord=float("inf")))
            return peak if peak == peak else float("inf")

    def forward_c(self, x: torch.Tensor, out: torch.Tensor) -> None:
        if self.cplan is None:
            raise K.SavsrError("this plan has no C-side launch list")
        if not (x.is_cuda and out.is_cuda and x.is_contiguous() and out.is_contiguous() and x.dtype == out.dtype == torch.float32):
            raise ValueError("savsr_forward takes contiguous fp32 CUDA tensors")
        if tuple(x.shape) != tuple(self.x_in.shape) or tuple(out.shape) != tuple(self.out.shape):
            raise ValueError(f"plan built for {tuple(self.x_in.shape)} -> {tuple(self.out.shape)}, got {tuple(x.shape)} -> {tuple(out.shape)}")
        with torch.cuda.device(self.device):
            K.check(self.lib.savsr_forward(self.cplan.handle, x.data_ptr(), out.data_ptr(), self._stream().cuda_stream))

    def release(self) -> None:
        self.graph = None
        self.cplan = None
        self.ops.clear()
        self._keep.clear()
        self._pack_src.clear()
        self.tap_bufs.clear()
        for name in ("arena_lr_t", "x_in", "out", "table", "lr"):
            if hasattr(self, name):
                setattr(self, name, None)
        self.nbytes = 0

    def read_tap(self, name: str) -> torch.Tensor:
        return self.tap_bufs[name]
```

Measured before the change: 268.7.

## Split OSA assemble into attention and tiled assemble kernels; retile mask kernels

Splits OSA weight assembly into a per-sample attention kernel and a smem-staged assemble kernel that caches the bank weights in shared memory. It then loops over many samples and writes the packed weights with 16-byte stores. It also adds load batching to the CA residual kernel, a multi-pixel variant of mask_conv16, and a shared-memory tiled mask_final bilinear kernel, plus a shared pooling helper. This adds one more launch and new indexing assumptions (for example ci a multiple of 64 and co a multiple of 4), which could break odd configurations.

New measurement: 271.8, median of 6. +1.2%, better.

```diff
diff --git a/savsr_b200/csrc/common.cuh b/savsr_b200/csrc/common.cuh
--- a/savsr_b200/csrc/common.cuh
+++ b/savsr_b200/csrc/common.cuh
@@ -51,7 +51,7 @@
 enum AttrBit { kAttrIgemm = 0 , kAttrBigk = 8, kAttrKsta = 9, kAttrSatuHr = 10, kAttrOsaLinear = 11,
                kAttrFused = 12, kAttrBigk128 = 13, kAttrSatuHrBf16 = 14, kAttrWgrad = 15, kAttrWgradBatched = 16,
                kAttrOsaAssembleTrain = 17, kAttrOsaUnfoldBwd = 18, kAttrOsaChain = 19, kAttrOsaMatvec = 20 ,
-               kAttrCaBackward = 23 };
+               kAttrCaBackward = 23, kAttrOsaAssemble = 24 };
 template <class F>
 inline int ensure_smem_attr(savsr_ctx* ctx, int bit, F func, size_t bytes) {
   if (ctx->attr_mask & (1u << bit)) return 0;
diff --git a/savsr_b200/csrc/small_ops.cu b/savsr_b200/csrc/small_ops.cu
--- a/savsr_b200/csrc/small_ops.cu
+++ b/savsr_b200/csrc/small_ops.cu
@@ -39,29 +39,45 @@
 
 __device__ __forceinline__ float sigmoidf_(float x) { return 1.f / (1.f + expf(-x)); }
 
-constexpr int kOsaThreads = 1024;
-__global__ void __launch_bounds__(kOsaThreads) osa_pool_kernel(const __grid_constant__ OsaLaunch L) {
+constexpr int kStageAhead = 8;
+template <class Load, class Store>
+__device__ __forceinline__ void stage_smem(int n, Load load, Store store) {
+  for (int i0 = threadIdx.x; i0 < n; i0 += kStageAhead * blockDim.x) {
+    float v[kStageAhead];
+#pragma unroll
+    for (int u = 0; u < kStageAhead; ++u) { const int i = i0 + u * blockDim.x; v[u] = i < n ? load(i) : 0.f; }
+#pragma unroll
+    for (int u = 0; u < kStageAhead; ++u) { const int i = i0 + u * blockDim.x; if (i < n) store(i, v[u]); }
+  }
+}
+
+constexpr int kPoolThreads = 1024;
+__device__ __forceinline__ float pool_channel_sum(const float* src, int npart, float (&red)[16][64]) {
+  const int ch = threadIdx.x & 63, part = threadIdx.x >> 6;
+  float a0 = 0.f, a1 = 0.f;
+  int q = part;
+  for (; q + 16 < npart; q += 32) { a0 += src[q * kC + ch]; a1 += src[(q + 16) * kC + ch]; }
+  if (q < npart) a0 += src[q * kC + ch];
+  red[part][ch] = a0 + a1;
+  __syncthreads();
+  float sum = 0.f;
+  if (part == 0) {
+#pragma unroll
+    for (int k = 0; k < 16; ++k) sum += red[k][ch];
+  }
+  return sum;
+}
+
+__global__ void __launch_bounds__(kPoolThreads) osa_pool_kernel(const __grid_constant__ OsaLaunch L) {
   pdl_wait();
   pdl_trigger();
   const savsr_osa_params& c = L.c[blockIdx.z];
   const int s = blockIdx.x, n = blockIdx.y;
   if (s * 64 >= c.ci) return;
   __shared__ float red[16][64];
-  const int ch = threadIdx.x & 63, part = threadIdx.x >> 6;
-  const float* src = c.pool[s] + static_cast<long>(n) * L.npart * kC;
-  float a0 = 0.f, a1 = 0.f;
-  int q = part;
-  for (; q + 16 < L.npart; q += 32) { a0 += src[q * kC + ch]; a1 += src[(q + 16) * kC + ch]; }
-  if (q < L.npart) a0 += src[q * kC + ch];
-  red[part][ch] = a0 + a1;
-  __syncthreads();
+  const float sum = pool_channel_sum(c.pool[s] + static_cast<long>(n) * L.npart * kC, L.npart, red);
   float* vin = c.scratch + static_cast<long>(n) * osa_scratch_stride(c.ci);
-  if (part == 0) {
-    float sum = 0.f;
-#pragma unroll
-    for (int k = 0; k < 16; ++k) sum += red[k][ch];
-    vin[2 + s * 64 + ch] = sum / static_cast<float>(L.npix);
-  }
+  if (threadIdx.x < 64) vin[2 + s * 64 + threadIdx.x] = sum / static_cast<float>(L.npix);
   if (s == 0 && threadIdx.x == 0) { vin[0] = L.inv_h; vin[1] = L.inv_w; }
 }
 
@@ -105,55 +121,45 @@
   }
 }
 
-constexpr int kAsmMaxSamples = 8;
-__global__ void __launch_bounds__(256) osa_assemble_kernel(const __grid_constant__ OsaLaunch L) {
+constexpr int kAttThreads = 1024;
+__global__ void __launch_bounds__(kAttThreads) osa_attention_kernel(const __grid_constant__ OsaLaunch L) {
+  pdl_wait();
+  pdl_trigger();
   const savsr_osa_params& c = L.c[blockIdx.y];
-  __shared__ float z_s[kAsmMaxSamples][32];
-  __shared__ float att_s[kAsmMaxSamples][64 * SAVSR_MAX_SRC + 64 + 9 + 8];
-  const int per = (L.batch + gridDim.z - 1) / gridDim.z;
-  const int n0 = blockIdx.z * per, n1 = min(L.batch, n0 + per);
-  if (n0 >= n1 || blockIdx.x * blockDim.x >= c.co * c.ci) return;
-  const int ns = n1 - n0;
+  const int n = blockIdx.x;
+  __shared__ float z_s[32];
+  __shared__ float att_s[64 * SAVSR_MAX_SRC + 64 + 9 + 8];
   const int warp = threadIdx.x >> 5, lane = threadIdx.x & 31;
-  const int stride = osa_scratch_stride(c.ci);
   const int nout = c.ci + c.co + 9 + 8;
-  for (int a = warp; a < c.att; a += 8) {
-    float wr[10];
-#pragma unroll
-    for (int j = 0; j < 10; ++j) wr[j] = lane + 32 * j < c.ci ? __ldg(c.fc_w + a * c.ci + lane + 32 * j) : 0.f;
-    const float bs = c.bn_scale[a], bh = c.bn_shift[a];
-    for (int n = 0; n < ns; ++n) {
-      const float* v2 = c.scratch + static_cast<long>(n0 + n) * stride + osa_off_v2(c.ci);
-      float acc = 0.f;
-#pragma unroll
-      for (int j = 0; j < 10; ++j) if (lane + 32 * j < c.ci) acc += wr[j] * v2[lane + 32 * j];
-#pragma unroll
-      for (int off = 16; off >= 1; off >>= 1) acc += __shfl_xor_sync(0xffffffffu, acc, off);
-      if (lane == 0) z_s[n][a] = fmaxf(acc * bs + bh, 0.f);
-    }
-  }
-  __syncthreads();
-  for (int j = threadIdx.x; j < nout; j += blockDim.x) {
-    const float* w;
-    float b;
-    if (j < c.ci) { w = c.ch_w + j * c.att; b = c.ch_b[j]; }
-    else if (j < c.ci + c.co) { w = c.fl_w + (j - c.ci) * c.att; b = c.fl_b[j - c.ci]; }
-    else if (j < c.ci + c.co + 9) { w = c.sp_w + (j - c.ci - c.co) * c.att; b = c.sp_b[j - c.ci - c.co]; }
-    else { w = c.kn_w + (j - c.ci - c.co - 9) * c.att; b = c.kn_b[j - c.ci - c.co - 9]; }
-    float wv[32];
-#pragma unroll
-    for (int a = 0; a < 32; ++a) wv[a] = a < c.att ? __ldg(w + a) : 0.f;
-    const bool sig = j < c.ci + c.co + 9;
-    for (int n = 0; n < ns; ++n) {
-      float acc = b;
-#pragma unroll
-      for (int a = 0; a < 32; ++a) if (a < c.att) acc += wv[a] * z_s[n][a];
-      att_s[n][j] = sig ? sigmoidf_(acc) : acc;
-    }
-  }
-  __syncthreads();
-  if (threadIdx.x < ns) {
-    float* ka = att_s[threadIdx.x] + c.ci + c.co + 9;
+  float* scratch = c.scratch + static_cast<long>(n) * osa_scratch_stride(c.ci);
+  if (warp < c.att) {
+    const float* v2 = scratch + osa_off_v2(c.ci);
+    float acc = 0.f;
+#pragma unroll
+    for (int j = 0; j < 10; ++j) if (lane + 32 * j < c.ci) acc += __ldg(c.fc_w + warp * c.ci + lane + 32 * j) * v2[lane + 32 * j];
+#pragma unroll
+    for (int off = 16; off >= 1; off >>= 1) acc += __shfl_xor_sync(0xffffffffu, acc, off);
+    if (lane == 0) z_s[warp] = fmaxf(acc * c.bn_scale[warp] + c.bn_shift[warp], 0.f);
+  }
+  const int j = threadIdx.x;
+  const float* w = nullptr;
+  float acc = 0.f;
+  if (j < c.ci) { w = c.ch_w + j * c.att; acc = c.ch_b[j]; }
+  else if (j < c.ci + c.co) { w = c.fl_w + (j - c.ci) * c.att; acc = c.fl_b[j - c.ci]; }
+  else if (j < c.ci + c.co + 9) { w = c.sp_w + (j - c.ci - c.co) * c.att; acc = c.sp_b[j - c.ci - c.co]; }
+  else if (j < nout) { w = c.kn_w + (j - c.ci - c.co - 9) * c.att; acc = c.kn_b[j - c.ci - c.co - 9]; }
+  float wv[32];
+#pragma unroll
+  for (int a = 0; a < 32; ++a) wv[a] = w && a < c.att ? __ldg(w + a) : 0.f;
+  __syncthreads();
+  if (j < nout) {
+#pragma unroll
+    for (int a = 0; a < 32; ++a) if (a < c.att) acc += wv[a] * z_s[a];
+    att_s[j] = j < c.ci + c.co + 9 ? sigmoidf_(acc) : acc;
+  }
+  __syncthreads();
+  if (threadIdx.x == 0) {
+    float* ka = att_s + c.ci + c.co + 9;
     float mx = ka[0];
     for (int k = 1; k < 8; ++k) mx = fmaxf(mx, ka[k]);
     float e[8], sum = 0.f;
@@ -161,39 +167,78 @@
     for (int k = 0; k < 8; ++k) ka[k] = e[k] / sum;
   }
   __syncthreads();
-  if (blockIdx.x == 0) {
-    for (int r = threadIdx.x; r < ns * nout; r += blockDim.x) {
-      const int n = r / nout, j = r - n * nout;
-      c.scratch[static_cast<long>(n0 + n) * stride + osa_off_att(c.ci) + j] = att_s[n][j];
-    }
-  }
-  const int idx = blockIdx.x * blockDim.x + threadIdx.x;
-  if (idx >= c.co * c.ci) return;
-  const int i = idx % c.ci, o = idx / c.ci;
-  float bk[8][9];
+  if (j < nout) scratch[osa_off_att(c.ci) + j] = att_s[j];
+}
+
+constexpr int kAsmThreads = 288;
+constexpr int kAsmRow = 73;
+constexpr int kAsmTile = 32;
+constexpr int kAsmAtt = 88;
+constexpr size_t kAsmSmem = 8 * 32 * kAsmRow * sizeof(float);
+__global__ void __launch_bounds__(kAsmThreads, 2) osa_assemble_kernel(const __grid_constant__ OsaLaunch L) {
+  extern __shared__ float bank_s[];
+  __shared__ float att_s[kAsmTile][kAsmAtt];
+  const savsr_osa_params& c = L.c[blockIdx.z];
+  const int s = blockIdx.y;
+  if (s * 64 >= c.ci) return;
+  const int ob = blockIdx.x % (c.co / 4), split = blockIdx.x / (c.co / 4), nsplit = gridDim.x / (c.co / 4);
+  const int per = (L.batch + nsplit - 1) / nsplit;
+  const int n0 = split * per, n1 = min(L.batch, n0 + per);
+  if (n0 >= n1) return;
   const long per_k = static_cast<long>(c.co) * c.ci * 9;
-#pragma unroll
-  for (int k = 0; k < 8; ++k) {
-    const float* src = c.bank + k * per_k + (static_cast<long>(o) * c.ci + i) * 9;
-#pragma unroll
-    for (int t = 0; t < 9; ++t) bk[k][t] = __ldg(src + t);
-  }
-  const int s = i >> 6, kk = i & 63;
+  pdl_wait();
+  constexpr int kLd = 8;
+#pragma unroll 1
+  for (int f0 = threadIdx.x; f0 < 8 * 4 * 144; f0 += kLd * kAsmThreads) {
+    float4 v[kLd];
+#pragma unroll
+    for (int u = 0; u < kLd; ++u) {
+      const int f = f0 + u * kAsmThreads, k = f / 576, ol = (f / 144) & 3, g = (f % 144) * 4;
+      v[u] = __ldg(reinterpret_cast<const float4*>(c.bank + k * per_k + (static_cast<long>(ob * 4 + ol) * c.ci + s * 64) * 9 + g));
+    }
+#pragma unroll
+    for (int u = 0; u < kLd; ++u) {
+      const int f = f0 + u * kAsmThreads, k = f / 576, ol = (f / 144) & 3, g = (f % 144) * 4;
+      float* d = bank_s + (k * 32 + ol * 8 + g / 72) * kAsmRow + g % 72;
+      d[0] = v[u].x; d[1] = v[u].y; d[2] = v[u].z; d[3] = v[u].w;
+    }
+  }
+  __syncthreads();
+  const int tap = threadIdx.x >> 5, lane = threadIdx.x & 31, ol = lane >> 3, chunk = lane & 7;
+  float bk[8][8];
+#pragma unroll
+  for (int k = 0; k < 8; ++k)
+#pragma unroll
+    for (int e = 0; e < 8; ++e) bk[k][e] = bank_s[(k * 32 + ol * 8 + chunk) * kAsmRow + e * 9 + tap];
+  const int o = ob * 4 + ol;
+  const int row = quad_row(o);
   const long sample_elems = static_cast<long>(c.co) * c.ci * 9;
-  const int row = quad_row(o);
-  const int inner = row * 64 + ((((kk >> 3) ^ (row & 7)) << 3) | (kk & 7));
-  for (int n = 0; n < ns; ++n) {
-    const float* att = att_s[n];
-    const float ca = att[i], fa = att[c.ci + o];
-    const float* sa = att + c.ci + c.co;
-    const float* ka = sa + 9;
-    uint16_t* dst = static_cast<uint16_t*>(c.packed) + (n0 + n) * sample_elems;
-#pragma unroll
-    for (int t = 0; t < 9; ++t) {
-      float acc = 0.f;
-#pragma unroll
-      for (int k = 0; k < 8; ++k) acc += ka[k] * bk[k][t];
-      dst[static_cast<long>(s * 9 + t) * 4096 + inner] = float_to_h(acc * sa[t] * ca * fa, L.fmt);
+  const long off = static_cast<long>(s * 9 + tap) * 4096 + row * 64 + ((chunk ^ (row & 7)) << 3);
+  const int stride = osa_scratch_stride(c.ci);
+  for (int t0 = n0; t0 < n1; t0 += kAsmTile) {
+    const int nt = min(kAsmTile, n1 - t0);
+    __syncthreads();
+    stage_smem(nt * 85, [&](int r) {
+      const int n = r / 85, j = r - n * 85;
+      const float* att = c.scratch + static_cast<long>(t0 + n) * stride + osa_off_att(c.ci);
+      return j < 64 ? att[s * 64 + j] : j < 68 ? att[c.ci + ob * 4 + j - 64] : att[c.ci + c.co + j - 68];
+    }, [&](int r, float x) { const int n = r / 85; att_s[n][r - n * 85] = x; });
+    __syncthreads();
+    for (int n = 0; n < nt; ++n) {
+      const float* a = att_s[n];
+      const float* ka = a + 77;
+      const float sa = a[68 + tap], fa = a[64 + ol];
+      float v[8];
+#pragma unroll
+      for (int e = 0; e < 8; ++e) {
+        float acc = 0.f;
+#pragma unroll
+        for (int k = 0; k < 8; ++k) acc += ka[k] * bk[k][e];
+        v[e] = acc * sa * a[chunk * 8 + e] * fa;
+      }
+      uint4 q;
+      q.x = pack_h2(v[0], v[1], L.fmt); q.y = pack_h2(v[2], v[3], L.fmt); q.z = pack_h2(v[4], v[5], L.fmt); q.w = pack_h2(v[6], v[7], L.fmt);
+      *reinterpret_cast<uint4*>(static_cast<uint16_t*>(c.packed) + (t0 + n) * sample_elems + off) = q;
     }
   }
 }
@@ -209,27 +254,15 @@
   int fmt;
   long npix;
 };
-__global__ void __launch_bounds__(1024) ca_vector_kernel(const CaParams p) {
+__global__ void __launch_bounds__(kPoolThreads) ca_vector_kernel(const CaParams p) {
   pdl_wait();
   pdl_trigger();
   __shared__ float red[16][64];
   __shared__ float mean[64];
   __shared__ float hid[4];
   const int n = blockIdx.x;
-  const int ch = threadIdx.x & 63, part = threadIdx.x >> 6;
-  const float* src = p.pool + static_cast<long>(n) * p.npart * kC;
-  float a0 = 0.f, a1 = 0.f;
-  int q = part;
-  for (; q + 16 < p.npart; q += 32) { a0 += src[q * kC + ch]; a1 += src[(q + 16) * kC + ch]; }
-  if (q < p.npart) a0 += src[q * kC + ch];
-  red[part][ch] = a0 + a1;
-  __syncthreads();
-  if (part == 0) {
-    float sum = 0.f;
-#pragma unroll
-    for (int k = 0; k < 16; ++k) sum += red[k][ch];
-    mean[ch] = sum / static_cast<float>(p.npix);
-  }
+  const float sum = pool_channel_sum(p.pool + static_cast<long>(n) * p.npart * kC, p.npart, red);
+  if (threadIdx.x < 64) mean[threadIdx.x] = sum / static_cast<float>(p.npix);
   __syncthreads();
   if (threadIdx.x < 4) {
     float a = p.b1[threadIdx.x];
@@ -255,131 +288,180 @@
   const uint4* tt = reinterpret_cast<const uint4*>(p.t + static_cast<long>(n) * p.npix * kC);
   const uint4* xx = reinterpret_cast<const uint4*>(p.x + static_cast<long>(n) * p.npix * kC);
   uint4* dd = reinterpret_cast<uint4*>(p.dst + static_cast<long>(n) * p.npix * kC);
-  for (long id = blockIdx.x * static_cast<long>(blockDim.x) + threadIdx.x; id < chunks;
-       id += static_cast<long>(gridDim.x) * blockDim.x) {
-    const int c0 = (id & 7) * 8;
-    const uint4 a = tt[id], b = xx[id];
-    uint4 o;
-    o.x = pack_h2(h_lo(b.x, p.fmt) + h_lo(a.x, p.fmt) * ys[c0 + 0], h_hi(b.x, p.fmt) + h_hi(a.x, p.fmt) * ys[c0 + 1], p.fmt);
-    o.y = pack_h2(h_lo(b.y, p.fmt) + h_lo(a.y, p.fmt) * ys[c0 + 2], h_hi(b.y, p.fmt) + h_hi(a.y, p.fmt) * ys[c0 + 3], p.fmt);
-    o.z = pack_h2(h_lo(b.z, p.fmt) + h_lo(a.z, p.fmt) * ys[c0 + 4], h_hi(b.z, p.fmt) + h_hi(a.z, p.fmt) * ys[c0 + 5], p.fmt);
-    o.w = pack_h2(h_lo(b.w, p.fmt) + h_lo(a.w, p.fmt) * ys[c0 + 6], h_hi(b.w, p.fmt) + h_hi(a.w, p.fmt) * ys[c0 + 7], p.fmt);
-    dd[id] = o;
-  }
-}
-
-template <bool kPool, bool kProj>
-__global__ void __launch_bounds__(256) mask_conv16_kernel(const float* __restrict__ in, const float* __restrict__ w,
-                                                          const float* __restrict__ b, const float* __restrict__ wf,
-                                                          float* __restrict__ out, int h2, int w2) {
+  constexpr int kResAhead = 4;
+  const long step = static_cast<long>(gridDim.x) * blockDim.x;
+  for (long id0 = blockIdx.x * static_cast<long>(blockDim.x) + threadIdx.x; id0 < chunks; id0 += kResAhead * step) {
+    uint4 a[kResAhead], b[kResAhead];
+#pragma unroll
+    for (int u = 0; u < kResAhead; ++u) {
+      const long id = id0 + u * step;
+      if (id < chunks) { a[u] = tt[id]; b[u] = xx[id]; }
+    }
+#pragma unroll
+    for (int u = 0; u < kResAhead; ++u) {
+      const long id = id0 + u * step;
+      if (id >= chunks) break;
+      const int c0 = (id & 7) * 8;
+      uint4 o;
+      o.x = pack_h2(h_lo(b[u].x, p.fmt) + h_lo(a[u].x, p.fmt) * ys[c0 + 0], h_hi(b[u].x, p.fmt) + h_hi(a[u].x, p.fmt) * ys[c0 + 1], p.fmt);
+      o.y = pack_h2(h_lo(b[u].y, p.fmt) + h_lo(a[u].y, p.fmt) * ys[c0 + 2], h_hi(b[u].y, p.fmt) + h_hi(a[u].y, p.fmt) * ys[c0 + 3], p.fmt);
+      o.z = pack_h2(h_lo(b[u].z, p.fmt) + h_lo(a[u].z, p.fmt) * ys[c0 + 4], h_hi(b[u].z, p.fmt) + h_hi(a[u].z, p.fmt) * ys[c0 + 5], p.fmt);
+      o.w = pack_h2(h_lo(b[u].w, p.fmt) + h_lo(a[u].w, p.fmt) * ys[c0 + 6], h_hi(b[u].w, p.fmt) + h_hi(a[u].w, p.fmt) * ys[c0 + 7], p.fmt);
+      dd[id] = o;
+    }
+  }
+}
+
+constexpr int kMaskThreads = 256;
+template <bool kPool, bool kProj, int kMaskPix>
+__global__ void __launch_bounds__(kMaskThreads) mask_conv16_kernel(const float* __restrict__ in, const float* __restrict__ w,
+                                                                   const float* __restrict__ b, const float* __restrict__ wf,
+                                                                   float* __restrict__ out, int h2, int w2) {
   __shared__ __align__(16) float w_s[9 * 16 * 16 + 36 * 4];
   __shared__ float wf_s[9 * 16];
-  for (int i = threadIdx.x; i < 9 * 256; i += blockDim.x) {
-    const int co = i & 15, ci = (i >> 4) & 15, tap = i >> 8;
-    w_s[i + (i >> 6) * 4] = w[(co * 16 + ci) * 9 + tap];
-  }
-  if (kProj) {
-    for (int i = threadIdx.x; i < 144; i += blockDim.x) wf_s[i] = wf[(i & 15) * 9 + (i >> 4)];
-  }
+  stage_smem(9 * 256, [&](int i) { return __ldg(w + (((i & 15) * 16 + ((i >> 4) & 15)) * 9 + (i >> 8))); },
+             [&](int i, float v) { w_s[i + (i >> 6) * 4] = v; });
+  if (kProj) stage_smem(144, [&](int i) { return __ldg(wf + (i & 15) * 9 + (i >> 4)); }, [&](int i, float v) { wf_s[i] = v; });
   __syncthreads();
   const int n = blockIdx.y;
   const int q = threadIdx.x & 3;
   const long npix2 = static_cast<long>(h2) * w2;
-  const long pix = blockIdx.x * static_cast<long>(blockDim.x >> 2) + (threadIdx.x >> 2);
-  const bool live = pix < npix2;
-  const int py = live ? pix / w2 : 0, px = live ? pix % w2 : 0;
-  float acc[16];
-#pragma unroll
-  for (int o = 0; o < 16; ++o) acc[o] = 0.f;
+  const long pix0 = blockIdx.x * static_cast<long>(kMaskThreads / 4 * kMaskPix) + (threadIdx.x >> 5) * 8 * kMaskPix + ((threadIdx.x & 31) >> 2);
+  long pix[kMaskPix];
+  bool live[kMaskPix];
+  int py[kMaskPix], px[kMaskPix];
+#pragma unroll
+  for (int j = 0; j < kMaskPix; ++j) {
+    pix[j] = pix0 + 8 * j;
+    live[j] = pix[j] < npix2;
+    py[j] = live[j] ? pix[j] / w2 : 0;
+    px[j] = live[j] ? pix[j] % w2 : 0;
+  }
+  float acc[kMaskPix][16];
+#pragma unroll
+  for (int j = 0; j < kMaskPix; ++j)
+#pragma unroll
+    for (int o = 0; o < 16; ++o) acc[j][o] = 0.f;
   const int wfull = 2 * w2;
   const float* base = kPool ? in + static_cast<long>(n) * (4 * npix2) * 16 : in + static_cast<long>(n) * npix2 * 16;
-#pragma unroll
+#pragma unroll 1
   for (int tap = 0; tap < 9; ++tap) {
-    const int sy = py + tap / 3 - 1, sx = px + tap % 3 - 1;
-    if (!live || sy < 0 || sy >= h2 || sx < 0 || sx >= w2) continue;
-    float4 a;
-    if (kPool) {
-      const float4 q0 = *reinterpret_cast<const float4*>(base + (static_cast<long>(2 * sy) * wfull + 2 * sx) * 16 + 4 * q);
-      const float4 q1 = *reinterpret_cast<const float4*>(base + (static_cast<long>(2 * sy) * wfull + 2 * sx + 1) * 16 + 4 * q);
-      const float4 q2 = *reinterpret_cast<const float4*>(base + (static_cast<long>(2 * sy + 1) * wfull + 2 * sx) * 16 + 4 * q);
-      const float4 q3 = *reinterpret_cast<const float4*>(base + (static_cast<long>(2 * sy + 1) * wfull + 2 * sx + 1) * 16 + 4 * q);
-      a.x = 0.25f * ((q0.x + q1.x) + (q2.x + q3.x)); a.y = 0.25f * ((q0.y + q1.y) + (q2.y + q3.y));
-      a.z = 0.25f * ((q0.z + q1.z) + (q2.z + q3.z)); a.w = 0.25f * ((q0.w + q1.w) + (q2.w + q3.w));
-    } else {
-      a = *reinterpret_cast<const float4*>(base + (static_cast<long>(sy) * w2 + sx) * 16 + 4 * q);
-    }
-    const float av[4] = {a.x, a.y, a.z, a.w};
+    float av[kMaskPix][4];
+#pragma unroll
+    for (int j = 0; j < kMaskPix; ++j) {
+      const int sy = py[j] + tap / 3 - 1, sx = px[j] + tap % 3 - 1;
+      float4 a = make_float4(0.f, 0.f, 0.f, 0.f);
+      if (live[j] && sy >= 0 && sy < h2 && sx >= 0 && sx < w2) {
+        if (kPool) {
+          const float4 q0 = __ldg(reinterpret_cast<const float4*>(base + (static_cast<long>(2 * sy) * wfull + 2 * sx) * 16 + 4 * q));
+          const float4 q1 = __ldg(reinterpret_cast<const float4*>(base + (static_cast<long>(2 * sy) * wfull + 2 * sx + 1) * 16 + 4 * q));
+          const float4 q2 = __ldg(reinterpret_cast<const float4*>(base + (static_cast<long>(2 * sy + 1) * wfull + 2 * sx) * 16 + 4 * q));
+          const float4 q3 = __ldg(reinterpret_cast<const float4*>(base + (static_cast<long>(2 * sy + 1) * wfull + 2 * sx + 1) * 16 + 4 * q));
+          a.x = 0.25f * ((q0.x + q1.x) + (q2.x + q3.x)); a.y = 0.25f * ((q0.y + q1.y) + (q2.y + q3.y));
+          a.z = 0.25f * ((q0.z + q1.z) + (q2.z + q3.z)); a.w = 0.25f * ((q0.w + q1.w) + (q2.w + q3.w));
+        } else {
+          a = __ldg(reinterpret_cast<const float4*>(base + (static_cast<long>(sy) * w2 + sx) * 16 + 4 * q));
+        }
+      }
+      av[j][0] = a.x; av[j][1] = a.y; av[j][2] = a.z; av[j][3] = a.w;
+    }
 #pragma unroll
     for (int c = 0; c < 4; ++c) {
       const float4* wr = reinterpret_cast<const float4*>(w_s + (tap * 16 + 4 * q + c) * 16 + (tap * 4 + q) * 4);
 #pragma unroll
       for (int o4 = 0; o4 < 4; ++o4) {
         const float4 wv = wr[o4];
-        acc[4 * o4 + 0] += av[c] * wv.x; acc[4 * o4 + 1] += av[c] * wv.y;
-        acc[4 * o4 + 2] += av[c] * wv.z; acc[4 * o4 + 3] += av[c] * wv.w;
+#pragma unroll
+        for (int j = 0; j < kMaskPix; ++j) {
+          acc[j][4 * o4 + 0] += av[j][c] * wv.x; acc[j][4 * o4 + 1] += av[j][c] * wv.y;
+          acc[j][4 * o4 + 2] += av[j][c] * wv.z; acc[j][4 * o4 + 3] += av[j][c] * wv.w;
+        }
       }
     }
   }
 #pragma unroll
-  for (int off = 2, cnt = 8; off >= 1; off >>= 1, cnt >>= 1) {
-    const bool upper = (q & off) != 0;
-#pragma unroll
-    for (int i = 0; i < cnt; ++i) {
-      const float send = upper ? acc[i] : acc[i + cnt];
-      const float keep = upper ? acc[i + cnt] : acc[i];
-      acc[i] = keep + __shfl_xor_sync(0xffffffffu, send, off);
-    }
-  }
-  float o4v[4];
-#pragma unroll
-  for (int i = 0; i < 4; ++i) o4v[i] = fmaxf(acc[i] + b[4 * q + i], 0.f);
-  if (!kProj) {
-    if (live) *reinterpret_cast<float4*>(out + (static_cast<long>(n) * npix2 + pix) * 16 + 4 * q) = make_float4(o4v[0], o4v[1], o4v[2], o4v[3]);
-  } else {
-    float d[9];
-#pragma unroll
-    for (int t = 0; t < 9; ++t) {
-      float v = 0.f;
-#pragma unroll
-      for (int i = 0; i < 4; ++i) v += wf_s[t * 16 + 4 * q + i] * o4v[i];
-      v += __shfl_xor_sync(0xffffffffu, v, 1);
-      v += __shfl_xor_sync(0xffffffffu, v, 2);
-      d[t] = v;
-    }
-    if (live && q < 3) {
-      float* dst = out + (static_cast<long>(n) * npix2 + pix) * 12 + 4 * q;
-      *reinterpret_cast<float4*>(dst) = q == 0 ? make_float4(d[0], d[1], d[2], d[3])
-                                     : q == 1 ? make_float4(d[4], d[5], d[6], d[7]) : make_float4(d[8], 0.f, 0.f, 0.f);
-    }
-  }
-}
-
+  for (int j = 0; j < kMaskPix; ++j) {
+#pragma unroll
+    for (int off = 2, cnt = 8; off >= 1; off >>= 1, cnt >>= 1) {
+      const bool upper = (q & off) != 0;
+#pragma unroll
+      for (int i = 0; i < cnt; ++i) {
+        const float send = upper ? acc[j][i] : acc[j][i + cnt];
+        const float keep = upper ? acc[j][i + cnt] : acc[j][i];
+        acc[j][i] = keep + __shfl_xor_sync(0xffffffffu, send, off);
+      }
+    }
+    float o4v[4];
+#pragma unroll
+    for (int i = 0; i < 4; ++i) o4v[i] = fmaxf(acc[j][i] + b[4 * q + i], 0.f);
+    if (!kProj) {
+      if (live[j]) *reinterpret_cast<float4*>(out + (static_cast<long>(n) * npix2 + pix[j]) * 16 + 4 * q) = make_float4(o4v[0], o4v[1], o4v[2], o4v[3]);
+    } else {
+      float d[9];
+#pragma unroll
+      for (int t = 0; t < 9; ++t) {
+        float v = 0.f;
+#pragma unroll
+        for (int i = 0; i < 4; ++i) v += wf_s[t * 16 + 4 * q + i] * o4v[i];
+        v += __shfl_xor_sync(0xffffffffu, v, 1);
+        v += __shfl_xor_sync(0xffffffffu, v, 2);
+        d[t] = v;
+      }
+      if (live[j] && q < 3) {
+        float* dst = out + (static_cast<long>(n) * npix2 + pix[j]) * 12 + 4 * q;
+        *reinterpret_cast<float4*>(dst) = q == 0 ? make_float4(d[0], d[1], d[2], d[3])
+                                        : q == 1 ? make_float4(d[4], d[5], d[6], d[7]) : make_float4(d[8], 0.f, 0.f, 0.f);
+      }
+    }
+  }
+}
+
+constexpr int kFinTile = 16;
+constexpr int kFinHalf = kFinTile / 2 + 3;
 __global__ void __launch_bounds__(256) mask_final_kernel(const float* __restrict__ d, const float* __restrict__ b,
                                                          float* __restrict__ mask, int h2, int w2) {
-  const int n = blockIdx.y;
+  __shared__ float d_s[9][kFinHalf][kFinHalf + 1];
+  const int n = blockIdx.z;
   const int H = 2 * h2, W = 2 * w2;
-  const long npix = static_cast<long>(H) * W;
-  const long pix = blockIdx.x * static_cast<long>(blockDim.x) + threadIdx.x;
-  if (pix >= npix) return;
-  const int py = pix / W, px = pix % W;
+  const int ty0 = blockIdx.y * kFinTile, tx0 = blockIdx.x * kFinTile;
+  const int hy0 = max(ty0 / 2 - 1, 0), hx0 = max(tx0 / 2 - 1, 0);
+  const int ny = min(h2 - hy0, kFinHalf), nx = min(w2 - hx0, kFinHalf);
   const float* base = d + static_cast<long>(n) * h2 * w2 * 12;
-  float acc = b[0];
-#pragma unroll
-  for (int tap = 0; tap < 9; ++tap) {
-    const int sy = py + tap / 3 - 1, sx = px + tap % 3 - 1;
-    if (sy < 0 || sy >= H || sx < 0 || sx >= W) continue;
-    float fy = 0.5f * (static_cast<float>(sy) + 0.5f) - 0.5f;
-    float fx = 0.5f * (static_cast<float>(sx) + 0.5f) - 0.5f;
+  for (int i = threadIdx.x; i < ny * nx * 3; i += blockDim.x) {
+    const int part = i % 3, cell = i / 3, r = cell / nx, cx = cell - r * nx;
+    const float4 v = __ldg(reinterpret_cast<const float4*>(base + (static_cast<long>(hy0 + r) * w2 + hx0 + cx) * 12) + part);
+    const float vv[4] = {v.x, v.y, v.z, v.w};
+#pragma unroll
+    for (int e = 0; e < 4; ++e)
+      if (4 * part + e < 9) d_s[4 * part + e][r][cx] = vv[e];
+  }
+  __syncthreads();
+  const int py = ty0 + (threadIdx.x >> 4), px = tx0 + (threadIdx.x & 15);
+  if (py >= H || px >= W) return;
+  int y0[3], y1[3], x0[3], x1[3];
+  float ly[3], lx[3];
+#pragma unroll
+  for (int u = 0; u < 3; ++u) {
+    float fy = 0.5f * (static_cast<float>(py + u - 1) + 0.5f) - 0.5f;
+    float fx = 0.5f * (static_cast<float>(px + u - 1) + 0.5f) - 0.5f;
     fy = fy < 0.f ? 0.f : fy;
     fx = fx < 0.f ? 0.f : fx;
-    const int y0 = static_cast<int>(fy), x0 = static_cast<int>(fx);
-    const int y1 = y0 + (y0 < h2 - 1 ? 1 : 0), x1 = x0 + (x0 < w2 - 1 ? 1 : 0);
-    const float ly = fy - y0, lx = fx - x0;
-    const float v00 = base[(static_cast<long>(y0) * w2 + x0) * 12 + tap], v01 = base[(static_cast<long>(y0) * w2 + x1) * 12 + tap];
-    const float v10 = base[(static_cast<long>(y1) * w2 + x0) * 12 + tap], v11 = base[(static_cast<long>(y1) * w2 + x1) * 12 + tap];
-    acc += (1.f - ly) * ((1.f - lx) * v00 + lx * v01) + ly * ((1.f - lx) * v10 + lx * v11);
-  }
-  mask[static_cast<long>(n) * npix + pix] = sigmoidf_(acc);
+    y0[u] = static_cast<int>(fy); x0[u] = static_cast<int>(fx);
+    y1[u] = y0[u] + (y0[u] < h2 - 1 ? 1 : 0); x1[u] = x0[u] + (x0[u] < w2 - 1 ? 1 : 0);
+    ly[u] = fy - y0[u]; lx[u] = fx - x0[u];
+    y0[u] -= hy0; y1[u] -= hy0; x0[u] -= hx0; x1[u] -= hx0;
+  }
+  float acc = b[0];
+#pragma unroll
+  for (int tap = 0; tap < 9; ++tap) {
+    const int u = tap / 3, v = tap % 3;
+    const int sy = py + u - 1, sx = px + v - 1;
+    if (sy < 0 || sy >= H || sx < 0 || sx >= W) continue;
+    const float v00 = d_s[tap][y0[u]][x0[v]], v01 = d_s[tap][y0[u]][x1[v]];
+    const float v10 = d_s[tap][y1[u]][x0[v]], v11 = d_s[tap][y1[u]][x1[v]];
+    acc += (1.f - ly[u]) * ((1.f - lx[v]) * v00 + lx[v] * v01) + ly[u] * ((1.f - lx[v]) * v10 + lx[v] * v11);
+  }
+  mask[static_cast<long>(n) * H * W + static_cast<long>(py) * W + px] = sigmoidf_(acc);
 }
 
 __device__ __forceinline__ float y_of_u8(int b, int g, int r) {
@@ -520,7 +602,7 @@
   L.nconvs = nconvs; L.batch = batch; L.npart = npart; L.npix = npix;
   L.inv_h = inv_scale_h; L.inv_w = inv_scale_w;
   L.fmt = ctx->fmt;
-  (void)launch_k(ctx->opt[SAVSR_OPT_PDL] != 0, osa_pool_kernel, dim3(max_ci / 64, batch, nconvs), dim3(kOsaThreads), 0, st, L);
+  (void)launch_k(ctx->opt[SAVSR_OPT_PDL] != 0, osa_pool_kernel, dim3(max_ci / 64, batch, nconvs), dim3(kPoolThreads), 0, st, L);
   const int lin_split = batch >= 12 ? 3 : (batch >= 4 ? 2 : 1);
   const size_t lin_smem = static_cast<size_t>((batch + lin_split - 1) / lin_split) * 2 * max_ci * sizeof(float);
   SAVSR_REQUIRE(lin_smem <= 200 * 1024, "savsr_osa_prologue: batch %d too large for the routing kernel's shared memory", batch);
@@ -560,9 +642,13 @@
   L.inv_h = inv_scale_h; L.inv_w = inv_scale_w;
   L.fmt = ctx->fmt;
   if (int rc = osa_prologue_front(ctx, convs, nconvs, batch, npart, npix, inv_scale_h, inv_scale_w, st)) return rc;
-  int asm_split = batch >= 16 ? 4 : (batch >= 6 ? 2 : 1);
-  while ((batch + asm_split - 1) / asm_split > kAsmMaxSamples) ++asm_split;
-  osa_assemble_kernel<<<dim3((64 * max_ci + 255) / 256, nconvs, asm_split), 256, 0, st>>>(L);
+  const bool pdl = ctx->opt[SAVSR_OPT_PDL] != 0;
+  (void)launch_k(pdl, osa_attention_kernel, dim3(batch, nconvs), dim3(kAttThreads), 0, st, L);
+  const int asm_blocks = 16 * (max_ci / 64) * nconvs;
+  int asm_split = 2 * ctx->sm_count / asm_blocks;
+  asm_split = asm_split < 1 ? 1 : (asm_split < batch ? asm_split : batch);
+  if (int rc = ensure_smem_attr(ctx, kAttrOsaAssemble, osa_assemble_kernel, kAsmSmem)) return rc;
+  (void)launch_k(pdl, osa_assemble_kernel, dim3(16 * asm_split, max_ci / 64, nconvs), dim3(kAsmThreads), kAsmSmem, st, L);
   SAVSR_CUDA(cudaGetLastError());
   return 0;
 }
@@ -585,7 +671,7 @@
   const long cap = 8L * ctx->sm_count / (arena->batch > 0 ? arena->batch : 1) + 1;
   if (blocks > cap) blocks = cap;
   if (arena->batch == 0) return 0;
-  (void)launch_k(ctx->opt[SAVSR_OPT_PDL] != 0, ca_vector_kernel, dim3(arena->batch), dim3(1024), 0, static_cast<cudaStream_t>(st), p);
+  (void)launch_k(ctx->opt[SAVSR_OPT_PDL] != 0, ca_vector_kernel, dim3(arena->batch), dim3(kPoolThreads), 0, static_cast<cudaStream_t>(st), p);
   (void)launch_k(ctx->opt[SAVSR_OPT_PDL] != 0, ca_scale_residual_kernel, dim3(static_cast<unsigned>(blocks), arena->batch), dim3(256), 0, static_cast<cudaStream_t>(st), p);
   SAVSR_CUDA(cudaGetLastError());
   return 0;
@@ -601,10 +687,17 @@
   cudaStream_t st = static_cast<cudaStream_t>(st_);
   const int h2 = height / 2, w2 = width / 2;
   const long npix2 = static_cast<long>(h2) * w2;
-  dim3 g2(static_cast<unsigned>((npix2 + 63) / 64), batch);
-  mask_conv16_kernel<true, false><<<g2, 256, 0, st>>>(in16, wa, ba, nullptr, half0, h2, w2);
-  mask_conv16_kernel<false, true><<<g2, 256, 0, st>>>(half0, wb, bb, wc, half1, h2, w2);
-  dim3 g1(static_cast<unsigned>((4 * npix2 + 255) / 256), batch);
+  const long blocks4 = (npix2 + kMaskThreads - 1) / kMaskThreads;
+  if (blocks4 * batch >= 2L * ctx->sm_count) {
+    dim3 g2(static_cast<unsigned>(blocks4), batch);
+    mask_conv16_kernel<true, false, 4><<<g2, kMaskThreads, 0, st>>>(in16, wa, ba, nullptr, half0, h2, w2);
+    mask_conv16_kernel<false, true, 4><<<g2, kMaskThreads, 0, st>>>(half0, wb, bb, wc, half1, h2, w2);
+  } else {
+    dim3 g2(static_cast<unsigned>((npix2 + kMaskThreads / 4 - 1) / (kMaskThreads / 4)), batch);
+    mask_conv16_kernel<true, false, 1><<<g2, kMaskThreads, 0, st>>>(in16, wa, ba, nullptr, half0, h2, w2);
+    mask_conv16_kernel<false, true, 1><<<g2, kMaskThreads, 0, st>>>(half0, wb, bb, wc, half1, h2, w2);
+  }
+  dim3 g1((width + kFinTile - 1) / kFinTile, (height + kFinTile - 1) / kFinTile, batch);
   mask_final_kernel<<<g1, 256, 0, st>>>(half1, bc, mask, h2, w2);
   SAVSR_CUDA(cudaGetLastError());
   return 0;
diff --git a/savsr_b200/engine.py b/savsr_b200/engine.py
--- a/savsr_b200/engine.py
+++ b/savsr_b200/engine.py
@@ -297,7 +297,7 @@
         inv_w = float(np.float32(1.0) / np.float32(self.scale[1]))
         lib, ctx, n, B = self.lib, self.ctx.handle, len(convs), self.B
         npart, npix = self.lr.tiles * 4, self.hp * self.wp
-        self._emit(lambda st: lib.savsr_osa_prologue(ctx, arr, n, B, npart, npix, inv_h, inv_w, st), launches=4, kind="osa_prologue",
+        self._emit(lambda st: lib.savsr_osa_prologue(ctx, arr, n, B, npart, npix, inv_h, inv_w, st), launches=5, kind="osa_prologue",
                    rec=lambda cp: lib.savsr_plan_add_osa_prologue(cp, arr, n, B, npart, npix, inv_h, inv_w))
 
     def _pool(self, key: str) -> int:
```
